# alperkartkaya2-afk/two-tower-augmented-with-adaptive-mimic-mechanism

Measured on AMD Instinct MI355X. Metric: training interactions/sec at 1/2/4/8 MI355X; Recall@20 parity vs CPU ref, higher is better.
Workload: dtype fp32

## Files before the change

two-tower-augmented-with-adaptive-mimic-mechanism_amd/csrc/gate.hip:

```cpp
#include <cstdlib>

#include "kernels.h"

namespace ttamm {

namespace {

typedef float f4v __attribute__((ext_vector_type(4)));
template <int D>
struct GateWaves {
    static constexpr int NW = D >= 128 ? 4 : 8;
    static constexpr int THREADS = 64 * NW;
};

__device__ __forceinline__ f4v ldg4(const float* p) { return *reinterpret_cast<const f4v*>(p); }
__device__ __forceinline__ f4v lds4(const float* p) { return *reinterpret_cast<const f4v*>(p); }
__device__ __forceinline__ void stg4(float* p, f4v v) { store_nt(p, make_float4(v[0], v[1], v[2], v[3])); }
__device__ __forceinline__ float sigmoid_(float x) { return 1.0f / (1.0f + __expf(-x)); }

template <int NO, int NK, int LD>
__device__ __forceinline__ void tile_gemm(const float* w_lds, int ob0, const f4v (&b)[NK], f4v (&acc)[NO], int li,
                                          int q) {
    f4v w[2][NO];
    const float* base = w_lds + (16 * ob0 + li) * LD + 4 * q;
// ... 37 lines not shown
                acc[ob] = __builtin_amdgcn_mfma_f32_16x16x4f32(w[cur][ob][r], b[t][r], acc[ob], 0, 0, 0);
        __builtin_amdgcn_sched_barrier(0);
    }
}

typedef __bf16 g_bf16x8 __attribute__((ext_vector_type(8)));
typedef __bf16 g_bf16x4 __attribute__((ext_vector_type(4)));
typedef float g_f32x8 __attribute__((ext_vector_type(8)));

__device__ __forceinline__ void split8(f4v a, f4v b, g_bf16x8& h, g_bf16x8& m, g_bf16x8& l) {
    const g_f32x8 x = {a[0], a[1], a[2], a[3], b[0], b[1], b[2], b[3]};
    h = __builtin_convertvector(x, g_bf16x8);
    const g_f32x8 r = x - __builtin_convertvector(h, g_f32x8);
    m = __builtin_convertvector(r, g_bf16x8);
    l = __builtin_convertvector(r - __builtin_convertvector(m, g_f32x8), g_bf16x8);
}

template <int NF>
__device__ __forceinline__ int xw_off(int t, int q, int f, int j) {
    return ((t * 4 + q) * NF + f) * 16 + j * 2;
}
__device__ __forceinline__ void xw_slot(int c, int& t, int& q, int& j) {
    t = c >> 5;
    const int r = c & 31;
    q = (r & 15) >> 2;
    j = ((r >> 4) << 2) | (r & 3);
}
template <int NF, int PLANE>
__device__ __forceinline__ void xw_store4(unsigned char* img, int t, int q, int f, int j0, f4v w) {
    const f4v hf = w;
    const g_bf16x4 h = __builtin_convertvector(hf, g_bf16x4);
    const f4v r = hf - __builtin_convertvector(h, f4v);
    const g_bf16x4 m = __builtin_convertvector(r, g_bf16x4);
    const g_bf16x4 l = __builtin_convertvector(r - __builtin_convertvector(m, f4v), g_bf16x4);
    const int off = xw_off<NF>(t, q, f, j0);
    *reinterpret_cast<g_bf16x4*>(img + off) = h;
    *reinterpret_cast<g_bf16x4*>(img + PLANE + off) = m;
    *reinterpret_cast<g_bf16x4*>(img + 2 * PLANE + off) = l;
}

template <int NO, int NT, int NF>
__device__ __forceinline__ void tile_gemm_x(const unsigned char* img, int ob0, const f4v* b, f4v (&acc)[NO], int li,
                                            int q) {
    constexpr int PLANE = NT * 4 * NF * 16;
#pragma unroll
    for (int t = 0; t < NT; ++t) {
        g_bf16x8 bh, bm, bl;
        split8(b[2 * t], b[2 * t + 1], bh, bm, bl);
        const unsigned char* base = img + xw_off<NF>(t, q, 16 * ob0 + li, 0);
#pragma unroll
        for (int ob = 0; ob < NO; ++ob) {
            const unsigned char* p = base + ob * 16 * 16;
            const g_bf16x8 ah = *reinterpret_cast<const g_bf16x8*>(p);
            const g_bf16x8 am = *reinterpret_cast<const g_bf16x8*>(p + PLANE);
            const g_bf16x8 al = *reinterpret_cast<const g_bf16x8*>(p + 2 * PLANE);
            acc[ob] = __builtin_amdgcn_mfma_f32_16x16x32_bf16(am, bm, acc[ob], 0, 0, 0);
            acc[ob] = __builtin_amdgcn_mfma_f32_16x16x32_bf16(al, bh, acc[ob], 0, 0, 0);
            acc[ob] = __builtin_amdgcn_mfma_f32_16x16x32_bf16(ah, bl, acc[ob], 0, 0, 0);
            acc[ob] = __builtin_amdgcn_mfma_f32_16x16x32_bf16(am, bh, acc[ob], 0, 0, 0);
            acc[ob] = __builtin_amdgcn_mfma_f32_16x16x32_bf16(ah, bm, acc[ob], 0, 0, 0);
            acc[ob] = __builtin_amdgcn_mfma_f32_16x16x32_bf16(ah, bh, acc[ob], 0, 0, 0);
        }
        __builtin_amdgcn_sched_barrier(0);
    }
}

template <int N>
__device__ __forceinline__ void zero(f4v (&a)[N]) {
#pragma unroll
    for (int i = 0; i < N; ++i) a[i] = f4v{0.f, 0.f, 0.f, 0.f};
}

template <int N>
__device__ __forceinline__ void load_row(f4v (&v)[N], const float* base, int64_t ld, int64_t row, int q) {
    const float* p = base + row * ld + 4 * q;
#pragma unroll
    for (int t = 0; t < N; ++t) v[t] = ldg4(p + 16 * t);
}

template <int D>
constexpr int slab_scratch() { return 8 * ((D < 96 ? 96 : D) + 4); }
template <int NO>
__device__ __forceinline__ void store_slab(float* scr, const f4v (&v)[NO], float* out, int64_t ld, int64_t row0,
                                           int64_t R, int lane) {
    constexpr int W = 16 * NO, LDW = W + 4, C4 = W / 4, PER = 8 * C4 / 64;
    static_assert((8 * C4) % 64 == 0, "slab scratch");
    const int li = lane & 15, q = lane >> 4;
#pragma unroll
    for (int half = 0; half < 2; ++half) {
        if ((li >> 3) == half) {
#pragma unroll
            for (int ob = 0; ob < NO; ++ob) *reinterpret_cast<f4v*>(scr + (li & 7) * LDW + 16 * ob + 4 * q) = v[ob];
        }
        __builtin_amdgcn_s_waitcnt(0xc07f);
        __builtin_amdgcn_wave_barrier();
#pragma unroll
        for (int k = 0; k < PER; ++k) {
            const int idx = lane + 64 * k, r = idx / C4, c = idx - r * C4;
            const f4v val = *reinterpret_cast<const f4v*>(scr + r * LDW + 4 * c);
            const int64_t grow = row0 + 8 * half + r;
            if (grow < R) stg4(out + grow * ld + 4 * c, val);
        }
        __builtin_amdgcn_s_waitcnt(0xc07f);
        __builtin_amdgcn_wave_barrier();
    }
}

template <int NO>
__device__ __forceinline__ void store_slab_xu(float* scr, const f4v (&v)[NO], float* out, int xu_li,
                                              bool pos_only, int64_t row0, int64_t R, int lane) {
    constexpr int W = 16 * NO, LDW = W + 4, C4 = W / 4, PER = 8 * C4 / 64;
    static_assert((8 * C4) % 64 == 0, "slab scratch");
    const int li = lane & 15, q = lane >> 4;
#pragma unroll
    for (int half = 0; half < 2; ++half) {
        if ((li >> 3) == half) {
#pragma unroll
            for (int ob = 0; ob < NO; ++ob) *reinterpret_cast<f4v*>(scr + (li & 7) * LDW + 16 * ob + 4 * q) = v[ob];
        }
        __builtin_amdgcn_s_waitcnt(0xc07f);
        __builtin_amdgcn_wave_barrier();
#pragma unroll
        for (int k = 0; k < PER; ++k) {
            const int idx = lane + 64 * k, r = idx / C4, c = idx - r * C4;
            const f4v val = *reinterpret_cast<const f4v*>(scr + r * LDW + 4 * c);
            const int64_t grow = row0 + 8 * half + r;
            const int u = __shfl(xu_li, 8 * half + r, 64);
            if (grow < R && (u >= 0 || !pos_only)) stg4(out + (int64_t)(u >= 0 ? u : ~u) * W + 4 * c, val);
        }
        __builtin_amdgcn_s_waitcnt(0xc07f);
        __builtin_amdgcn_wave_barrier();
    }
}

template <int N>
__device__ __forceinline__ void load_dt_row(f4v (&v)[N], const float* base, int64_t ld, const int64_t* xu, int D,
                                            int64_t row, int q) {
    if (xu) {
        const int64_t u = xu[row];
        load_row(v, base, D, u >= 0 ? u : ~u, q);
    } else {
        load_row(v, base, ld, row, q);
    }
}

template <int D, int HG, int NW_ = GateWaves<D>::NW>
struct GateCfg {
    static constexpr int TD = D / 16, TH = HG / 16, TE = 2 * D / 16;
    static constexpr int NW = NW_;
    static constexpr bool GG = D >= 128;
    static constexpr int SCR = slab_scratch<(D > HG ? D : HG)>();
    static constexpr int F_LD1 = 2 * D + 4, F_LD2 = HG + 4;
    static constexpr int F_LDS = HG * F_LD1 + (GG ? 0 : D * F_LD2) + HG + D;
    static constexpr int B_LD1 = D + 4, B_LD2 = HG + 4;
    static constexpr int B_G1T = GG ? 0 : HG * B_LD1;
    static constexpr int B_LDS = B_G1T + 2 * D * B_LD2;
    static_assert(D % 16 == 0 && HG % 16 == 0, "16-feature tiles");
    static_assert((F_LDS + NW * SCR) * 4 <= 163840 && (B_LDS + NW * SCR) * 4 <= 163840,
                  "the gate matrices must fit one CU's LDS");
    static constexpr int X1_BYTES = 3 * 2 * (2 * D) * HG;
    static constexpr int XF_BYTES = X1_BYTES + 4 * (D * F_LD2 + HG + D);
    static constexpr int XB_BYTES = X1_BYTES + 4 * (HG * B_LD1);
    static constexpr bool X_OK = !GG && (2 * D) % 32 == 0 && HG % 32 == 0 && XF_BYTES <= 163840 && XB_BYTES <= 163840;
};

__device__ __forceinline__ int gate_tower(const KArg(GateArgs) * ka, int& bidx) {
    bidx = blockIdx.x;
    if (ka->count > 1 && bidx >= ka->tw[0].blocks) {
        bidx -= ka->tw[0].blocks;
        return 1;
    }
    return 0;
}

template <int D, int HG, bool X, int NW>
__global__ __launch_bounds__(64 * NW) void gate_fwd_kernel(GateArgs) {
    using C = GateCfg<D, HG, NW>;
    constexpr int NT = 64 * NW;
    constexpr int NX = (2 * D) / 32;
    __shared__ __attribute__((aligned(16))) float lds[X ? C::XF_BYTES / 4 : C::F_LDS + NW * C::SCR];
    const KArg(GateArgs)* ka = (const KArg(GateArgs)*)(__builtin_amdgcn_kernarg_segment_ptr());
    int bidx;
    const KArg(GateTower)& T = ka->tw[gate_tower(ka, bidx)];
    float* g1s = lds;
// ... 19 lines not shown
#pragma unroll
    for (int e0 = 0; e0 < N1; e0 += NT) {
        const int e = e0 + (int)threadIdx.x;
        if (e < N1) {
            const int i = e / (2 * D / 4), c = 4 * (e % (2 * D / 4));
            const f4v w = ldg4(T.G1 + (int64_t)i * 2 * D + c);
            if constexpr (X) {
                int t, q4, j;
                xw_slot(c, t, q4, j);
                xw_store4<HG, C::X1_BYTES / 3>(img, t, q4, i, j, w);
            } else {
                *reinterpret_cast<f4v*>(g1s + i * C::F_LD1 + c) = w;
            }
        }
    }
    if constexpr (!C::GG) {
#pragma unroll
        for (int e0 = 0; e0 < N2; e0 += NT) {
            const int e = e0 + (int)threadIdx.x;
            if (e < N2) {
                const int i = e / (HG / 4), c = 4 * (e % (HG / 4));
                *reinterpret_cast<f4v*>(g2s + i * C::F_LD2 + c) = ldg4(T.G2 + (int64_t)i * HG + c);
            }
        }
    }
    for (int e = threadIdx.x; e < HG + D; e += NT) c1s[e] = e < HG ? T.c1[e] : T.c2[e - HG];
    __syncthreads();
    for (; s < nslab; s += stride) {
        const int64_t row = s * 16 + li;
        const bool ok = row < R;
        f4v a[C::TD];
        if (T.table) load_row(a, T.table, D, arow, q);
        const int xu_li = T.xu && ok ? (int)T.xu[row] : 0;
        f4v z[C::TH];
        zero(z);
        if constexpr (X) tile_gemm_x<C::TH, NX, HG>(img, 0, ef, z, li, q);
        else tile_gemm<C::TH, C::TE, C::F_LD1>(g1s, 0, ef, z, li, q);
        f4v nx[C::GG ? 1 : C::TE];
        int64_t arow_n = 0;
        const int64_t sn = s + stride;
        if (!C::GG && sn < nslab) {
            const int64_t rn = sn * 16 + li < R ? sn * 16 + li : R - 1;
            load_row(nx, T.ef, 2 * D, rn, q);
            if (T.table) arow_n = T.idx[rn];
        }
#pragma unroll
        for (int ob = 0; ob < C::TH; ++ob) {
            const f4v c1 = lds4(c1s + 16 * ob + 4 * q);
#pragma unroll
            for (int r = 0; r < 4; ++r) {
                const float v = z[ob][r] + c1[r];
                z[ob][r] = v > 0.f ? v : 0.f;
            }
            if ((X || (kDevKnobs && ka->direct)) && ok && !(kDevKnobs && ka->ablate)) stg4(T.z + row * HG + 16 * ob + 4 * q, z[ob]);
        }
        if (!(X || (kDevKnobs && ka->direct)) && !(kDevKnobs && ka->ablate)) store_slab<C::TH>(scr, z, T.z, HG, s * 16, R, lane);
        f4v x[C::TD];
        zero(x);
        if constexpr (C::GG) tile_gemm_g<C::TD, C::TH, HG>(T.G2, 0, z, x, li, q);
        else tile_gemm<C::TD, C::TH, C::F_LD2>(g2s, 0, z, x, li, q);
        if (!(X || (kDevKnobs && ka->direct)) && !(kDevKnobs && ka->ablate)) {
#pragma unroll
            for (int ob = 0; ob < C::TD; ++ob) {
                const f4v c2 = lds4(c2s + 16 * ob + 4 * q);
#pragma unroll
                for (int r = 0; r < 4; ++r) x[ob][r] = sigmoid_(x[ob][r] + c2[r]);
            }
            store_slab<C::TD>(scr, x, T.g, D, s * 16, R, lane);
#pragma unroll
            for (int ob = 0; ob < C::TD; ++ob) {
                const f4v e = ef[ob], f = ef[C::TD + ob];
#pragma unroll
                for (int r = 0; r < 4; ++r) x[ob][r] = x[ob][r] * e[r] + (1.0f - x[ob][r]) * f[r];
            }
            if (T.xu) {
                store_slab_xu<C::TD>(scr, a, T.a, xu_li, true, s * 16, R, lane);
                const bool neg = xu_li < 0;
#pragma unroll
                for (int ob = 0; ob < C::TD; ++ob)
#pragma unroll
                    for (int r = 0; r < 4; ++r) x[ob][r] = neg ? x[ob][r] + a[ob][r] : x[ob][r];
                store_slab_xu<C::TD>(scr, x, T.t, xu_li, false, s * 16, R, lane);
            } else {
                store_slab<C::TD>(scr, x, T.t, T.ld_t, s * 16, R, lane);
                if (T.table) {
                    store_slab<C::TD>(scr, a, T.a, T.ld_t, s * 16, R, lane);
#pragma unroll
                    for (int ob = 0; ob < C::TD; ++ob)
#pragma unroll
                        for (int r = 0; r < 4; ++r) x[ob][r] = x[ob][r] + a[ob][r];
                }
                if (T.aug) store_slab<C::TD>(scr, x, T.aug, D, s * 16, R, lane);
            }
        }
        if ((X || (kDevKnobs && ka->direct)) && ok && !(kDevKnobs && ka->ablate)) {
            const int64_t xu = xu_li;
            float* tdst = T.xu ? T.t + (xu >= 0 ? xu : ~xu) * D : T.t + row * T.ld_t;
            float* adst = T.xu ? (xu >= 0 ? T.a + xu * D : nullptr) : (T.table ? T.a + row * T.ld_t : nullptr);
#pragma unroll
            for (int ob = 0; ob < C::TD; ++ob) {
                const int col = 16 * ob + 4 * q;
                const f4v c2 = lds4(c2s + col);
                const f4v e = ef[ob], f = ef[C::TD + ob];
                f4v g, tt;
#pragma unroll
                for (int r = 0; r < 4; ++r) {
                    g[r] = sigmoid_(x[ob][r] + c2[r]);
                    tt[r] = g[r] * e[r] + (1.0f - g[r]) * f[r];
                }
                stg4(T.g + row * D + col, g);
                f4v aug = tt;
                if (T.table) {
#pragma unroll
                    for (int r = 0; r < 4; ++r) aug[r] = tt[r] + a[ob][r];
                }
                stg4(tdst + col, T.xu && xu < 0 ? aug : tt);
                if (adst) stg4(adst + col, a[ob]);
                if (T.aug) stg4(T.aug + row * D + col, aug);
            }
        }
        if constexpr (C::GG) {
            if (sn < nslab) {
                const int64_t rn = sn * 16 + li < R ? sn * 16 + li : R - 1;
                load_row(ef, T.ef, 2 * D, rn, q);
                if (T.table) arow = T.idx[rn];
            }
        } else if (sn < nslab) {
#pragma unroll
            for (int t = 0; t < C::TE; ++t) ef[t] = nx[t];
            arow = arow_n;
        }
    }
}

template <int D, int HG, bool X, int NW>
__global__ __launch_bounds__(64 * NW) void gate_bwd_kernel(GateArgs) {
    using C = GateCfg<D, HG, NW>;
    constexpr int NT = 64 * NW;
    constexpr int NX = HG / 32;
    __shared__ __attribute__((aligned(16))) float lds[X ? C::XB_BYTES / 4 : C::B_LDS + NW * C::SCR];
    const KArg(GateArgs)* ka = (const KArg(GateArgs)*)(__builtin_amdgcn_kernarg_segment_ptr());
    int bidx;
    const KArg(GateTower)& T = ka->tw[gate_tower(ka, bidx)];
    unsigned char* img = reinterpret_cast<unsigned char*>(lds);
    float* g2t = X ? reinterpret_cast<float*>(img + C::X1_BYTES) : lds;
    float* g1t = lds + C::B_G1T;
    float* scr = lds + C::B_LDS + (threadIdx.x >> 6) * C::SCR;
    const int lane = threadIdx.x & 63, wave = threadIdx.x >> 6;
    const int li = lane & 15, q = lane >> 4;
    const int64_t R = T.R;
    const int64_t nslab = (R + 15) / 16;
    const int64_t stride = (int64_t)T.blocks * NW;
    constexpr int N2 = D * (HG / 4), N1 = HG * (2 * D / 4);
    auto stage_g2t = [&]() {
#pragma unroll
        for (int e0 = 0; e0 < N2; e0 += NT) {
            const int e = e0 + (int)threadIdx.x;
            if (e < N2) {
                const int d = e / (HG / 4), j = 4 * (e % (HG / 4));
                const f4v v = ldg4(T.G2 + (int64_t)d * HG + j);
#pragma unroll
                for (int i = 0; i < 4; ++i) g2t[(j + i) * C::B_LD1 + d] = v[i];
            }
        }
    };
    if constexpr (C::GG) {
        for (int64_t s0 = (int64_t)bidx * NW; s0 < nslab; s0 += stride) {
            const int64_t s = s0 + wave;
            const bool has = s < nslab;
            const int64_t row = s * 16 + li;
            const bool ok = has && row < R;
            const int64_t rr = ok ? row : R - 1;
            f4v d[C::TD], g[C::TD], dz[C::TH];
            {
                f4v ef[C::TE];
                load_dt_row(d, T.dT, T.ld_dT, T.xu, D, rr, q);
                load_row(ef, T.ef, 2 * D, rr, q);
                load_row(g, T.g, D, rr, q);
                stage_g2t();
                __syncthreads();
                if (has) {
                    f4v dq[C::TD];
#pragma unroll
                    for (int t = 0; t < C::TD; ++t)
#pragma unroll
                        for (int r = 0; r < 4; ++r) {
                            const float dg = d[t][r] * ef[t][r] - d[t][r] * ef[C::TD + t][r];
                            dq[t][r] = dg * (1.0f - g[t][r]) * g[t][r];
                        }
                    if (!(kDevKnobs && ka->ablate)) store_slab<C::TD>(scr, dq, T.dq, D, s * 16, R, lane);
                    f4v zr[C::TH];
                    load_row(zr, T.z, HG, rr, q);
                    zero(dz);
                    tile_gemm<C::TH, C::TD, C::B_LD1>(g2t, 0, dq, dz, li, q);
#pragma unroll
                    for (int ob = 0; ob < C::TH; ++ob)
#pragma unroll
                        for (int r = 0; r < 4; ++r) dz[ob][r] = zr[ob][r] > 0.f ? dz[ob][r] : 0.f;
                    if (!(kDevKnobs && ka->ablate)) store_slab<C::TH>(scr, dz, T.dz, HG, s * 16, R, lane);
                }
            }
// ... 192 lines not shown
```

two-tower-augmented-with-adaptive-mimic-mechanism_amd/csrc/gemm.hip:

```cpp
#include <cstdlib>
#include <cstring>
#include <type_traits>

#include "kernels.h"

#ifndef TTAMM_GEMM_ABLATE
#define TTAMM_GEMM_ABLATE 0
#endif
#ifndef TTAMM_B16_ABLATE
#define TTAMM_B16_ABLATE 0
#endif

namespace ttamm {

typedef float f32x16 __attribute__((ext_vector_type(16)));
typedef float f32x8 __attribute__((ext_vector_type(8)));
typedef __bf16 bf16x8 __attribute__((ext_vector_type(8)));

namespace {


constexpr int BK = 16;
constexpr int SK = BK + 4;
constexpr int kThreads = 256;
constexpr int kWgradMaxRowsPerSplit = 1024;

__device__ __forceinline__ float sigmoidf_(float x) { return 1.0f / (1.0f + __expf(-x)); }
__device__ __forceinline__ bool aligned16(const void* p) { return (reinterpret_cast<uintptr_t>(p) & 15u) == 0; }
__device__ __forceinline__ bf16x8 pack_bf16(float4 a, float4 b) {
    const f32x8 v = {a.x, a.y, a.z, a.w, b.x, b.y, b.z, b.w};
    return __builtin_convertvector(v, bf16x8);
}
__device__ __forceinline__ float f4get(const float4& v, int q) {
    return q == 0 ? v.x : q == 1 ? v.y : q == 2 ? v.z : v.w;
}

__device__ __forceinline__ int clamp_col(int c, int ld) { return max(0, min(c, ld - 4)); }
__device__ __forceinline__ float4 raw4(const float* rp, int c, int ld) {
    return *reinterpret_cast<const float4*>(rp + clamp_col(c, ld));
}
__device__ __forceinline__ float4 mask4(float4 v, int c, int lim, int ld, int ones, bool ok) {
    const bool same = clamp_col(c, ld) == c;
    float t[4] = {v.x, v.y, v.z, v.w};
#pragma unroll
    for (int e = 0; e < 4; ++e) {
        const int ce = c + e;
        t[e] = (ok && same && ce < lim) ? t[e] : ((ok && ce == ones) ? 1.0f : 0.f);
    }
    return make_float4(t[0], t[1], t[2], t[3]);
}

template <int BM_, int BN_, int WAVES_M_, int WAVES_N_, bool A_KMAJ_, bool B_KMAJ_, int MF_ = 32>
struct Cfg {
    static constexpr int BM = BM_, BN = BN_, WAVES_M = WAVES_M_, WAVES_N = WAVES_N_, MF = MF_;
    static constexpr bool A_KMAJ = A_KMAJ_, B_KMAJ = B_KMAJ_;
    static constexpr int TM = BM / WAVES_M, TN = BN / WAVES_N;
    static constexpr int I = TM / MF, J = TN / MF;
    static constexpr int NR = MF == 32 ? 16 : 4;
    static constexpr int A_F4 = BM * BK / 4, B_F4 = BN * BK / 4;
    static constexpr int A_LOADS = (A_F4 + kThreads - 1) / kThreads;
    static constexpr int B_LOADS = (B_F4 + kThreads - 1) / kThreads;
    static constexpr int A_STAGE = A_KMAJ ? BK * BM : BM * SK;
    static constexpr int B_STAGE = B_KMAJ ? BK * BN : BN * SK;
    static constexpr int STAGE = 2 * (A_STAGE + B_STAGE);
    static constexpr int CLD = BN + 4;
    static constexpr int EPI_ROWS = WAVES_M >= 2 ? BM / 2 : (I > 1 ? (I + 1) / 2 * MF : BM);
    static constexpr int EPI_PHASES = (BM + EPI_ROWS - 1) / EPI_ROWS;
    static constexpr int EPI = EPI_ROWS * CLD;
    static constexpr int KIDX = A_KMAJ ? 2 * kWgradMaxRowsPerSplit : 0;
    static constexpr int LDS = (STAGE + KIDX) > EPI ? (STAGE + KIDX) : EPI;
    static_assert(WAVES_M * WAVES_N == 4, "4 waves per block");
    static_assert(MF == 32 || MF == 16, "MFMA block edge");
    static_assert(TM % MF == 0 && TN % MF == 0, "wave tile must be a multiple of the MFMA block");
    static_assert(WAVES_M == 1 || WAVES_M % EPI_PHASES == 0, "epilogue slices must hold whole wave rows");
};

__device__ __forceinline__ float4 ld4(const float* p) { return *reinterpret_cast<const float4*>(p); }
__device__ __forceinline__ void st4(float* p, float4 v) { store_nt(p, v); }

constexpr float kSeluAlpha = 1.6732632423543772848170429916717f;
constexpr float kSeluScale = 1.0507009873554804934193349852946f;
__device__ __forceinline__ float act_fwd(int act, float z) {
    switch (act) {
        case TTAMM_ACT_GELU: return z * 0.5f * (1.0f + erff(z * 0.70710678118654752440f));
        case TTAMM_ACT_TANH: return tanhf(z);
        case TTAMM_ACT_SELU: return z > 0.f ? z * kSeluScale : (expf(z) - 1.0f) * (kSeluAlpha * kSeluScale);
// ... 1142 lines not shown
        for (int i = 0; i < 4; ++i) {
            const int br = wm * 128 + i * 32;
            if (br < row_lo || br >= row_lo + kB16EpiRows) continue;
#pragma unroll
            for (int j = 0; j < 2; ++j)
#pragma unroll
                for (int r = 0; r < 16; ++r) {
                    const int rr = br - row_lo + (r & 3) + 8 * (r >> 2) + 4 * h;
                    Cs[rr * kB16Cld + wn * 64 + j * 32 + li] = acc[i][j][r];
                }
        }
        __syncthreads();
        if constexpr (E == EPI_HIDDEN) {
            constexpr int C4 = kB16N / 4;
            constexpr int RSTEP = kB16Threads / C4;
            static_assert(C4 % 2 == 0, "lane pairs hold 8-column groups");
            const int c4 = tid % C4, r0 = tid / C4;
            const int col = n0 + c4 * 4;
            if (r0 < RSTEP && col < ((N + 7) & ~7)) {
                const float4 bias4 = (P.bias && col < N) ? ld4(P.bias + col) : make_float4(0.f, 0.f, 0.f, 0.f);
                const float4 z4 = make_float4(0.f, 0.f, 0.f, 0.f);
#pragma unroll 2
                for (int rr = r0; rr < kB16EpiRows; rr += 2 * RSTEP) {
                    const int rb_ = rr + RSTEP;
                    const int ra = m0 + row_lo + rr, rb = m0 + row_lo + rb_;
                    const bool in_b = rb_ < kB16EpiRows;
                    epilogue_hidden_pair(P, ld4(Cs + rr * kB16Cld + c4 * 4), in_b ? ld4(Cs + rb_ * kB16Cld + c4 * 4) : z4, bias4,
                                         0, ra, rb, ra < M && col < N, in_b && rb < M && col < N, col);
                }
            }
        } else {
            constexpr int C4 = kB16N / 4;
            constexpr int RSTEP = kB16Threads / C4;
            const int c4 = tid % C4, r0 = tid / C4;
            const int col = n0 + c4 * 4;
            if (col < N) {
                const bool has_bias = (E == EPI_STORE || E == EPI_HIDDEN || E == EPI_GATE_HIDDEN || E == EPI_GATE_OUT) &&
                                      P.bias != nullptr;
                const float4 bias4 = has_bias ? ld4(P.bias + col) : make_float4(0.f, 0.f, 0.f, 0.f);
    #pragma unroll 2
                for (int rr = r0; rr < kB16EpiRows; rr += RSTEP) {
                    const int row = m0 + row_lo + rr;
    #if TTAMM_B16_ABLATE == 1
                    if (row < M) st4(P.C + (int64_t)row * P.ldc + col, ld4(Cs + rr * kB16Cld + c4 * 4));
    #else
                    if (row < M) epilogue4<E>(P, ld4(Cs + rr * kB16Cld + c4 * 4), bias4, 0, row, col);
    #endif
                }
            }
        }
        __syncthreads();
    }
}

__global__ void to_bf16_kernel(const float* __restrict__ src, int64_t rows, int cols, int64_t ld_src,
                               uint16_t* __restrict__ dst, int64_t ld_dst) {
    const int64_t total = rows * ld_dst;
    for (int64_t i = (int64_t)blockIdx.x * blockDim.x + threadIdx.x; i < total; i += (int64_t)gridDim.x * blockDim.x) {
        const int64_t r = i / ld_dst;
        const int c = (int)(i - r * ld_dst);
        const __bf16 v = (__bf16)(c < cols ? src[r * ld_src + c] : 0.f);
        dst[i] = __builtin_bit_cast(uint16_t, v);
    }
}

__global__ void to_planes_kernel(const float* __restrict__ src, int64_t rows, int cols, int64_t ld_src,
                                 uint16_t* __restrict__ dst, int64_t ld_dst, int kc) {
    const int64_t per_row = (int64_t)kc * 4;
    const int64_t total = rows * per_row;
    for (int64_t i = (int64_t)blockIdx.x * blockDim.x + threadIdx.x; i < total; i += (int64_t)gridDim.x * blockDim.x) {
        const int64_t r = i / per_row;
        const int g = (int)(i - r * per_row), c0 = 4 * g;
        float v[4];
#pragma unroll
        for (int e = 0; e < 4; ++e) v[e] = c0 + e < cols ? src[r * ld_src + c0 + e] : 0.f;
        uint2 w[3];
        split_bf16<3>(make_float4(v[0], v[1], v[2], v[3]), w);
        uint16_t* o = dst + r * ld_dst + (c0 >> 4) * 48 + (c0 & 15);
#pragma unroll
        for (int pl = 0; pl < 3; ++pl) *reinterpret_cast<uint2*>(o + 16 * pl) = w[pl];
    }
}

__global__ void wgrad_reduce_kernel(WgradBatch batch, int64_t total) {
    const KArg(WgradBatch)* kb = (const KArg(WgradBatch)*)(__builtin_amdgcn_kernarg_segment_ptr());
    const int64_t gid = (int64_t)blockIdx.x * blockDim.x + threadIdx.x;
    if (gid >= total) return;
    int64_t off = gid;
    int pi = 0;
    for (; pi < kb->count; ++pi) {
        const int64_t sz = (int64_t)kb->p[pi].M * (kb->p[pi].N + 1);
        if (off < sz) break;
        off -= sz;
    }
    const KArg(WgradProblem)& P = kb->p[pi];
    const int Mo = P.M;
    const int64_t plane = (int64_t)(P.N + 1) * Mo;
    const int n = (int)(off / Mo), m = (int)(off - (int64_t)n * Mo);
    float s = 0.f;
    const float* src = P.slab + off;
    int sp = 0;
    for (; sp + 8 <= P.splits; sp += 8) {
        float v[8];
#pragma unroll
        for (int i = 0; i < 8; ++i) v[i] = src[(int64_t)(sp + i) * plane];
#pragma unroll
        for (int i = 0; i < 8; ++i) s += v[i];
    }
    for (; sp < P.splits; ++sp) s += src[(int64_t)sp * plane];
    if (n < P.N) P.grad_w[(int64_t)m * P.N + n] = s;
    else if (P.grad_b) P.grad_b[m] = s;
}

template <class CF, int E, bool BF>
int launch_one(GemmBatch& b, hipStream_t s) {
    int tiles = 0;
    for (int i = 0; i < b.count; ++i) {
        GemmProblem& p = b.p[i];
        p.tiles_m = (int)ceil_div(p.M, CF::BM);
        p.tiles_n = (int)ceil_div(p.N, CF::BN);
        if (p.k_split <= 0) p.k_split = p.K;
        p.tile_begin = tiles;
        tiles += p.tiles_m * p.tiles_n * (int)ceil_div(p.K, p.k_split);
    }
    b.total_tiles = tiles;
    if (tiles == 0) return TTAMM_OK;
    hipLaunchKernelGGL((gemm_kernel<CF, E, BF>), dim3(tiles), dim3(kThreads), 0, s, b);
    TTAMM_LAUNCH_CHECK();
    return TTAMM_OK;
}

template <class CX, int E, int PL>
int launch_one_x(GemmBatch& b, hipStream_t s) {
    int tiles = 0;
    for (int i = 0; i < b.count; ++i) {
        GemmProblem& p = b.p[i];
        p.tiles_m = (int)ceil_div(p.M, CX::BM);
        p.tiles_n = (int)ceil_div(p.N, CX::BN);
        if (p.k_split <= 0) p.k_split = p.K;
        p.tile_begin = tiles;
        tiles += p.tiles_m * p.tiles_n * (int)ceil_div(p.K, p.k_split);
    }
    b.total_tiles = tiles;
    if (tiles == 0) return TTAMM_OK;
    hipLaunchKernelGGL((gemm_x_kernel<CX, E, PL>), dim3(tiles), dim3(kThreads), 0, s, b);
    TTAMM_LAUNCH_CHECK();
    return TTAMM_OK;
}
template <class CX, int PL>
int dispatch_epi_x(GemmBatch& b, hipStream_t s) {
    switch (b.p[0].epi) {
        case EPI_STORE: return launch_one_x<CX, EPI_STORE, PL>(b, s);
        case EPI_HIDDEN: return launch_one_x<CX, EPI_HIDDEN, PL>(b, s);
        case EPI_GATE_HIDDEN: return launch_one_x<CX, EPI_GATE_HIDDEN, PL>(b, s);
        case EPI_GATE_OUT: return launch_one_x<CX, EPI_GATE_OUT, PL>(b, s);
        case EPI_DGRAD_RELU: return launch_one_x<CX, EPI_DGRAD_RELU, PL>(b, s);
        case EPI_DGRAD_GATE_EF: return launch_one_x<CX, EPI_DGRAD_GATE_EF, PL>(b, s);
        case EPI_DGRAD_HIDDEN: return launch_one_x<CX, EPI_DGRAD_HIDDEN, PL>(b, s);
        default: return fail(TTAMM_E_INVALID, "gemm: unknown epilogue");
    }
}
template <int BM, int BN, int WM, int WN, bool AK, bool BK>
int dispatch_x(GemmBatch& b, hipStream_t s) {
    static const bool adeep2 = [] {
        const char* e = dev_env("TTAMM_GEMM_ADEEP");
        return e && e[0] == '2';
    }();
    if (b.p[0].bf16) return dispatch_epi_x<XCfg<BM, BN, WM, WN, AK, BK, 32>, 1>(b, s);
    if (adeep2 || AK || BK) return dispatch_epi_x<XCfg<BM, BN, WM, WN, AK, BK, 16>, 3>(b, s);
    return dispatch_epi_x<XCfg<BM, BN, WM, WN, AK, BK, 16, 3>, 3>(b, s);
}
int pick_tile_n(const GemmBatch& b, bool narrow, bool bf16) {
    static const bool legacy = [] {
        const char* e = dev_env("TTAMM_GEMM_TILES");
        return e && std::strcmp(e, "legacy") == 0;
    }();
    int maxN = 0;
    for (int i = 0; i < b.count; ++i) maxN = b.p[i].N > maxN ? b.p[i].N : maxN;
    if (maxN <= 96) return 96;
    if (legacy) return narrow ? 96 : 192;
    (void)bf16;
    static const int kNarrow[] = {96, 128};
    static const int kWide[] = {192, 128, 96};
    const int* c = narrow ? kNarrow : kWide;
    const int nc = narrow ? 2 : 3;
    int best = c[0];
    int64_t best_cols = -1;
    for (int j = 0; j < nc; ++j) {
        int64_t cols = 0;
        for (int i = 0; i < b.count; ++i) cols += ceil_div(b.p[i].M, 128) * ceil_div(b.p[i].N, c[j]) * c[j];
        if (best_cols < 0 || cols < best_cols) best_cols = cols, best = c[j];
    }
    return best;
}
// ... 164 lines not shown
                                 : (const void*)gemm_kernel<WgradNarrow, EPI_STORE, false>)
                          : cls == 0 ? (const void*)gemm_x_kernel<WgradNarrowX, EPI_STORE, 3>
                          : cls == 1 ? (const void*)gemm_x_kernel<WgradWideX, EPI_STORE, 3>
                                     : (const void*)gemm_x_kernel<Wgrad128X, EPI_STORE, 3>;
    if (hipOccupancyMaxActiveBlocksPerMultiprocessor(&per_cu, k, kThreads, 0) != hipSuccess || per_cu < 1) per_cu = 1;
    cached[exact][cls] = cus * per_cu;
    return cached[exact][cls];
}
constexpr int kWgradTileN[kWgradClasses] = {96, 192, 128, 128};
}

void wgrad_rows_per_split(const WgradShape* shapes, int n, int rps[kWgradClasses]) {
    if (const char* e = dev_env("TTAMM_WGRAD_ROWS_PER_SPLIT")) {
        const int v = std::atoi(e);
        if (v >= BK && v <= kWgradMaxRowsPerSplit && v % BK == 0) {
            for (int c = 0; c < kWgradClasses; ++c) rps[c] = v;
            return;
        }
    }
    const bool exact = exact_mfma();
    const double us_per_row[kWgradClasses] = {0.11, 0.14, 0.12, 0.12};
    const double hbm_us_per_byte = 1.0 / 5.0e6;
    for (int c = 0; c < kWgradClasses; ++c) {
        int best = 512;
        double best_cost = -1.0;
        for (int r = 128; r <= kWgradMaxRowsPerSplit; r += 32) {
            int64_t tiles = 0;
            double slab_bytes = 0.0;
            for (int i = 0; i < n; ++i) {
                if (shapes[i].R <= 0 || wgrad_class(shapes[i].M) != c) continue;
                const int64_t splits = ceil_div(shapes[i].R, r);
                tiles += ceil_div(shapes[i].N + 1, 128) * ceil_div(shapes[i].M, kWgradTileN[c]) * splits;
                slab_bytes += 2.0 * 4.0 * (double)splits * shapes[i].M * (shapes[i].N + 1);
            }
            if (tiles == 0) break;
            const double cost = (double)ceil_div(tiles, wgrad_slots(c, exact)) * r * us_per_row[c] +
                                slab_bytes * hbm_us_per_byte;
            if (best_cost < 0.0 || cost < best_cost) {
                best_cost = cost;
                best = r;
            }
        }
        rps[c] = best;
        if constexpr (kDevKnobs) {
            char name[] = "TTAMM_WGRAD_RPS0";
            name[sizeof(name) - 2] = (char)('0' + c);
            if (const char* e = dev_env(name)) {
                const int v = std::atoi(e);
                if (v >= BK && v <= kWgradMaxRowsPerSplit && v % BK == 0) rps[c] = v;
            }
        }
    }
}

size_t wgrad_slab_floats(int R, int M, int N, int rps) {
    const int splits = R > 0 ? (int)ceil_div(R, rps) : 1;
    return (size_t)splits * M * (N + 1);
}

int wgrad_class(int m_out) {
    static const bool all_narrow = dev_env("TTAMM_WGRAD_ALL_NARROW") != nullptr;
    static const bool legacy = [] {
        const char* e = dev_env("TTAMM_GEMM_TILES");
        return e && std::strcmp(e, "legacy") == 0;
    }();
    if (all_narrow || m_out <= 96) return 0;
    if (legacy) return 1;
    auto pad = [&](int bn) { return ceil_div(m_out, bn) * bn; };
    int best = 1;
    int64_t bp = pad(192);
    if (pad(256) < bp) best = 3, bp = pad(256);
    if (pad(128) < bp) best = 2, bp = pad(128);
    return best;
}

static bool wgrad_a3() {
    static const bool on = [] {
        const char* e = dev_env("TTAMM_WGRAD_ADEEP");
        return e && e[0] == '3';
    }();
    return on;
}

int launch_wgrad(WgradBatch& wb, hipStream_t s, void* const* ev) {
    GemmBatch g[kWgradClasses], gp[kWgradClasses];
    std::memset(g, 0, sizeof(g));
    std::memset(gp, 0, sizeof(gp));
    const bool bf = wb.count > 0 && wb.p[0].bf16;
    const bool exact = exact_mfma();
    const char* e256 = dev_env("TTAMM_BF16_WGRAD256");
    const bool w256 = e256 && e256[0] == '1';
    auto cfg_of = [&](int cls) {
        if (exact) return cls == 0 ? 0 : 1;
        if (bf && w256 && cls >= 2) return 3;
        return cls == 3 ? 2 : cls;
    };
    auto flush = [&](GemmBatch& b, int cfg, bool planes = false) -> int {
        if (b.count == 0) return TTAMM_OK;
        int rc;
        if (planes && bf) {
            rc = cfg == 1 ? launch_one_x<WgradWideX32A16, EPI_STORE, 1>(b, s)
                          : launch_one_x<Wgrad128X32A16, EPI_STORE, 1>(b, s);
        } else if (planes) {
            rc = cfg == 0   ? launch_one_x<WgradNarrowXP, EPI_STORE, 3>(b, s)
                 : cfg == 1 ? launch_one_x<WgradWideXP, EPI_STORE, 3>(b, s)
                            : launch_one_x<Wgrad128XP, EPI_STORE, 3>(b, s);
        } else if (exact) {
            rc = cfg ? (bf ? launch_one<WgradWide, EPI_STORE, true>(b, s) : launch_one<WgradWide, EPI_STORE, false>(b, s))
                     : (bf ? launch_one<WgradNarrow, EPI_STORE, true>(b, s) : launch_one<WgradNarrow, EPI_STORE, false>(b, s));
        } else if (bf) {
            rc = cfg == 0   ? launch_one_x<WgradNarrowX32, EPI_STORE, 1>(b, s)
                 : cfg == 1 ? launch_one_x<WgradWideX32, EPI_STORE, 1>(b, s)
                 : cfg == 3 ? launch_one_x<Wgrad256X32, EPI_STORE, 1>(b, s)
                            : launch_one_x<Wgrad128X32, EPI_STORE, 1>(b, s);
        } else {
            rc = cfg == 0   ? (wgrad_a3() ? launch_one_x<WgradNarrowXA3, EPI_STORE, 3>(b, s)
                                          : launch_one_x<WgradNarrowX, EPI_STORE, 3>(b, s))
                 : cfg == 1 ? launch_one_x<WgradWideX, EPI_STORE, 3>(b, s)
                            : launch_one_x<Wgrad128X, EPI_STORE, 3>(b, s);
        }
        std::memset(&b, 0, sizeof(b));
        return rc;
    };
    int64_t total = 0;
    for (int i = 0; i < wb.count; ++i) {
        WgradProblem& w = wb.p[i];
        TTAMM_REQUIRE(w.rows_per_split > 0 && w.rows_per_split % BK == 0 && w.rows_per_split <= kWgradMaxRowsPerSplit,
                      "wgrad: rows_per_split must be a multiple of 16 and at most 1024");
        TTAMM_REQUIRE(w.bf16 == wb.p[0].bf16, "wgrad: the batch must share one matmul precision");
        w.splits = w.R > 0 ? (int)ceil_div(w.R, w.rows_per_split) : 1;
        total += (int64_t)w.M * (w.N + 1);
        if (w.R <= 0) {
            TTAMM_HIP(hipMemsetAsync(w.slab, 0, sizeof(float) * w.M * (w.N + 1), s));
            continue;
        }
        TTAMM_REQUIRE(w.ld_x % 4 == 0 && w.ld_dy % 4 == 0 && ((uintptr_t)w.X | (uintptr_t)w.dY) % 16 == 0,
                      "wgrad: operands must be 16-byte aligned with leading dims % 4 == 0");
        GemmProblem p;
        std::memset(&p, 0, sizeof(p));
        p.A = w.X;
        p.a_idx = w.x_idx;
        p.lda = w.ld_x;
        p.a_kmaj = 1;
        p.a_cols = w.N;
        p.B = w.dY;
        p.ldb = w.ld_dy;
        p.b_kn = 1;
        p.b_colsum = 0;
        p.a_ones_col = w.N;
        p.M = w.N + 1;
        p.N = w.M;
        p.K = w.R;
        p.k_split = w.rows_per_split;
        p.epi = EPI_STORE;
        p.C = w.slab;
        p.ldc = w.M;
        p.slab_stride = (int64_t)(w.N + 1) * w.M;
        p.keep_prob = 1.f;
        p.inv_keep = 1.f;
        p.bf16 = w.bf16;
        const int cfg = cfg_of(wgrad_class(w.M));
        bool planes = w.X3p != nullptr && !exact && !bf && w.ld_x3 % 8 == 0 && (uintptr_t)w.X3p % 16 == 0 &&
                      w.ld_x3 >= 48 * ceil_div(w.N, 16);
        if (planes) {
            p.A3p = w.X3p;
            p.lda3 = w.ld_x3;
        }
        if (!exact && bf) {
            p.b_colsum = 1;
            p.a_ones_col = -1;
            p.M = w.N;
        }
        if (bf && w.X16 && (cfg == 1 || cfg == 2) && w.ld_x16 % 8 == 0 && w.ld_x16 >= 8 * ceil_div(w.N, 8) &&
            (uintptr_t)w.X16 % 16 == 0) {
            planes = true;
            p.A16 = w.X16;
            p.lda16 = w.ld_x16;
        }
        GemmBatch& gb = planes ? gp[cfg] : g[cfg];
        if (gb.count == kMaxGemmProblems) {
            const int rc = flush(gb, cfg, planes);
            if (rc) return rc;
        }
        gb.p[gb.count++] = p;
    }
    int rc;
    bool any_wide = false;
    for (int c = 1; c < kWgradClasses; ++c) any_wide = any_wide || g[c].count > 0 || gp[c].count > 0;
    const bool timed = ev && ev[0] && ev[1] && any_wide;
    static const bool narrow_first = dev_env("TTAMM_WGRAD_WIDE_FIRST") == nullptr;
    if (narrow_first && ((rc = flush(g[0], 0)) || (rc = flush(gp[0], 0, true)))) return rc;
    if (timed) TTAMM_HIP(hipEventRecord((hipEvent_t)ev[0], s));
    for (int c = 1; c < kWgradClasses; ++c)
        if ((rc = flush(gp[c], c, true)) || (rc = flush(g[c], c))) return rc;
    if (timed) TTAMM_HIP(hipEventRecord((hipEvent_t)ev[1], s));
    if (!narrow_first && ((rc = flush(g[0], 0)) || (rc = flush(gp[0], 0, true)))) return rc;
    if (total > 0) {
        hipLaunchKernelGGL(wgrad_reduce_kernel, dim3((unsigned)ceil_div(total, 256)), dim3(256), 0, s, wb, total);
        TTAMM_LAUNCH_CHECK();
    }
    return TTAMM_OK;
}

}
```

two-tower-augmented-with-adaptive-mimic-mechanism_amd/csrc/kernels.h:

```cpp
#pragma once

#include "common.h"

namespace ttamm {

enum Epilogue : int {
    EPI_STORE = 0,
    EPI_HIDDEN = 1,
    EPI_GATE_HIDDEN = 2,
    EPI_GATE_OUT = 3,
    EPI_DGRAD_RELU = 4,
    EPI_DGRAD_GATE_EF = 5,
    EPI_DGRAD_HIDDEN = 6,
};

struct GemmProblem {
    const float* A;
    const int64_t* a_idx;
    int64_t lda;
    const float* B;
    int64_t ldb;
    int b_kn;
    int M, N, K;
    int epi;
    float* C;
    int64_t ldc;
    const float* bias;
    const float* aux0;
    const float* aux1;
    const float* aux2;
    int64_t ld_aux0, ld_aux1, ld_aux2;
    float* out1;
    float* out2;
    float* out3;
    const float* table;
    const int64_t* idx;
    int64_t ld_out;
    int64_t ld_out2;
    float keep_prob;
    float inv_keep;
    const uint8_t* keep_mask;
    uint32_t rng_k0, rng_k1, rng_c2, rng_c3;
    const int64_t* row_key;
    int64_t key_base0, key_base1, key_split;
    int a_kmaj;
    int a_cols;
    int a_ones_col;
    int b_colsum;
    int k_split;
    int64_t slab_stride;
    int tile_begin;
    int tiles_m, tiles_n;
    int bf16;
    const uint16_t* A16;
    const uint16_t* B16;
    int64_t lda16;
    const uint16_t* A3p;
    int64_t lda3;
    int act;
    float* pre;
    uint8_t* mask_out;
};

constexpr int kMaxGemmProblems = 8;
struct GemmBatch {
    GemmProblem p[kMaxGemmProblems];
    int count;
    int total_tiles;
};

int launch_gemm(GemmBatch& batch, hipStream_t s);

int epoch_half_bits(int64_t n);
size_t route_scratch_bytes(int64_t n, int world);
int launch_route_rows(const int64_t* id0, int64_t n0, const int64_t* id1, int64_t n1, const int64_t* payload,
                      int64_t key0, int64_t key1, int world, int64_t* packed, int64_t* slot, int64_t* counts,
                      int64_t counts_ld, const uint32_t* status, void* scratch, size_t scratch_bytes, hipStream_t s);
void epoch_round_keys(uint64_t seed, int64_t epoch, uint32_t keys[4]);
int launch_epoch_batch(const int64_t* users, const int64_t* items, int64_t n, uint64_t seed, int64_t epoch,
                       int shuffle, int64_t start, int64_t count, int64_t* out_users, int64_t* out_items,
                       hipStream_t s);
int launch_to_bf16(const float* src, int64_t rows, int cols, int64_t ld_src, uint16_t* dst, int64_t ld_dst,
                   hipStream_t s);
int launch_to_planes(const float* src, int64_t rows, int cols, int64_t ld_src, uint16_t* dst, int64_t ld_dst,
                     hipStream_t s);

struct WgradProblem {
    const float* dY;
    int64_t ld_dy;
    const float* X;
    const int64_t* x_idx;
    int64_t ld_x;
    const uint16_t* X3p;
    int64_t ld_x3;
    const uint16_t* X16;
    int64_t ld_x16;
    int R, M, N;
    float* grad_w;
    float* grad_b;
    float* slab;
    int splits;
    int rows_per_split;
    int tile_begin;
    int tiles_m, tiles_n;
    int bf16;
};
constexpr int kMaxWgradProblems = 16;
static_assert(kMaxWgradProblems >= 2 * (TTAMM_MAX_LINEAR + 2), "both towers: every Linear + the gate's two");
struct WgradBatch {
    WgradProblem p[kMaxWgradProblems];
    int count;
    int total_blocks;
};
struct WgradShape {
    int64_t R;
    int M, N;
};
constexpr int kWgradClasses = 4;
int wgrad_class(int m_out);
void wgrad_rows_per_split(const WgradShape* shapes, int n, int rps[kWgradClasses]);
size_t wgrad_slab_floats(int R, int M, int N, int rows_per_split);
int launch_wgrad(WgradBatch& batch, hipStream_t s, void* const* ev = nullptr);

struct GateTower {
    int64_t R;
    const float* ef;
    const float* G1;
    const float* c1;
    const float* G2;
    const float* c2;
    float* z;
    float* g;
    float* t;
    float* a;
    int64_t ld_t;
    const float* table;
    const int64_t* idx;
    float* aug;
    const float* dT;
    int64_t ld_dT;
    const int64_t* xu;
    float* dq;
    float* dz;
    float* dEF;
    uint16_t* w16;
    int blocks;
};
struct GateArgs {
    GateTower tw[2];
    int count;
    int D, HG;
    int planes;
    int images_ready;
    int ablate;
    int direct;
};
bool gate_fused_supported(int D, int HG);
int launch_gate(GateArgs& a, bool backward, hipStream_t s);
bool gate16_supported(int D, int HG, int planes);
int64_t gate16_image_elems(int D, int HG, int planes);
int launch_gate16_prep(GateArgs& a, hipStream_t s);
int launch_gate16(GateArgs& a, bool backward, hipStream_t s);

int launch_renorm_rows(float* table, int64_t table_rows, int dim, const int64_t* idx, int64_t n, double max_norm,
                       int32_t* mark, int32_t tag, hipStream_t s, const int64_t* keys = nullptr,
                       int64_t key_split = 0, int key_phase = 0);
int launch_gather_rows(const float* table, int64_t table_rows, int dim, const int64_t* idx, int64_t n, float* out,
                       int64_t out_ld, hipStream_t s);

struct StageSeg {
    const int64_t* in;
    int64_t* out;
    int64_t n;
    int64_t rows;
    int64_t ld;
};
constexpr int kMaxStageSegs = 3;
struct StageArgs {
    StageSeg seg[kMaxStageSegs];
    int count;
    uint32_t* status;
    const int64_t* unit_counts;
    int64_t unit_ld;
    int unit_groups;
    int64_t unit_n;
    int64_t* unit_out;
};
int launch_stage_rows(const StageArgs& a, hipStream_t s);
int launch_add_rows(const float* x, int64_t ldx, const float* y, int64_t ldy, int64_t n, int dim, float* out,
                    int64_t ldo, hipStream_t s, const int64_t* xrow = nullptr);
int launch_scatter_add_rows(float* dst, int64_t dst_rows, int dim, const int64_t* idx, int64_t n, const float* x,
                            int64_t ldx, const float* y, int64_t ldy, const float* scale_dev, float scale,
                            int64_t skip_row, hipStream_t s);

constexpr uint32_t kStatusPoison =
    TTAMM_STATUS_SAMPLER_EXHAUSTED | TTAMM_STATUS_INDEX_OUT_OF_RANGE | TTAMM_STATUS_LOOKAHEAD_MISMATCH;
__device__ __forceinline__ bool step_poisoned(const uint32_t* status) {
    return status != nullptr && (*status & kStatusPoison) != 0u;
}
int launch_combine(const float* e, int64_t ld_e, const float* f, int64_t ld_f, const float* table,
                   int64_t table_rows, const int64_t* idx, int64_t n, int dim, float* t, float* a, int64_t ld_ta, float* aug,
                   hipStream_t s);
int launch_gate_mix(float* g, const float* ef, const float* table, const int64_t* idx, int64_t n, int dim, float* t,
                    float* a, int64_t ld_ta, float* aug, hipStream_t s);
int launch_pad_rows(const float* src, int64_t rows, int cols, int64_t ld_src, float* dst, int ld_dst,
                    hipStream_t s);
struct GatherSeg {
    const float* table;
    int64_t rows;
    int dim;
    const int64_t* idx;
    int64_t n;
    float* out;
    int64_t out_ld;
};
struct GatherSegs {
    GatherSeg seg[2];
    int count;
};
int launch_gather_rows_segs(const GatherSegs& g, hipStream_t s);
struct PadSeg {
    const float* src;
    int64_t rows;
    int cols;
    int64_t ld_src;
    float* dst;
    int ld_dst;
};
struct PadSegs {
    PadSeg seg[2];
    int count;
};
int launch_pad_rows_segs(const PadSegs& p, hipStream_t s);
int launch_mse(const float* x, const float* y, int64_t n, float* out, hipStream_t s);
int launch_gate_dq(const float* dT, int64_t ld_dT, const float* ef, const float* g, int64_t n, int dim,
                   float* dq, hipStream_t s);

struct ScoreArgs {
    int64_t B;
    int64_t Bg;
    int N;
    int D;
    const float* user_aug;
    const float* item_aug;
    const float* t_user;
    const float* t_item;
    const float* a_user;
    const float* a_item;
    int64_t ld_item;
    float lambda_u, lambda_i;
    int mimic;
    float* dT_user;
    float* dT_item;
    float* dA_user;
    float* dA_item;
    int dA_all;
    int neg_aug;
    int64_t ld_dti;
    const int64_t* item_slot;
    float* partials;
    int blocks;
    float inv_numel;
    const float* ib_du;
    const float* ib_dp;
    int64_t ib_ld;
};
int score_blocks(int64_t B, int D);
int launch_score_loss(const ScoreArgs& a, hipStream_t s);
struct EvalScoreArgs {
    int64_t B;
    int N;
    int D;
    const float* user_aug;
    const float* item_aug;
    int64_t ld_item;
    float* partials;
    int blocks;
    float* logits;
    int skip_pos;
};
int score_eval_check(int N, int D);
int launch_score_eval(const EvalScoreArgs& a, hipStream_t s);
int launch_eval_loss_finalize(const float* partials, int blocks, int64_t count, int64_t B, float* loss_out,
                              double* loss_accum, const uint32_t* status, hipStream_t s);
int launch_eval_loss_inbatch_finalize(const float* partials, int blocks, const float* ib_partials, int ib_blocks,
                                      int64_t count, int64_t B, float* loss_out, double* loss_accum,
                                      const uint32_t* status, hipStream_t s);
int launch_loss_finalize(const float* partials, int blocks, const float* ib_partials, int ib_blocks, int64_t bce_count,
                         int64_t B, int64_t Bg, int D, float lambda_u, float lambda_i, int mimic, const float* cal,
                         float lambda_cal, float* loss_out, double* loss_accum, const uint32_t* status, hipStream_t s);

struct InBatchArgs {
    const float* U;
    int64_t ldu, B;
    const float* P;
    int64_t ldp, Bc;
    int D;
    int64_t row_base;
    float inv_T;
    float* slab_u;
    float* slab_p;
    float* loss_part;
    float* dU;
    int64_t ld_du;
    float* dP;
    int64_t ld_dp;
    int rblk_u, rblk_p, splits_u, splits_p;
    int64_t cols_u, cols_p;
    const float* rmax;
    const float* rinv;
    float z_scale;
};
void inbatch_plan(int64_t B, int64_t Bc, InBatchArgs& a);
size_t inbatch_workspace_floats(int64_t B, int64_t Bc, int D, size_t* slab_u, size_t* slab_p, size_t* parts);
int launch_inbatch(InBatchArgs& a, hipStream_t s);
size_t inbatch_standalone_workspace_bytes(int64_t B, int64_t Bc, int D);
int inbatch_standalone(const float* U, int64_t B, int64_t ldu, const float* P, int64_t Bc, int64_t ldp, int D,
                       int64_t row_base, float inv_T, float* dU, int64_t ld_du, float* dP, int64_t ld_dp,
                       double* loss_sum, void* ws, size_t ws_bytes, hipStream_t s);
struct InBatchLossArgs {
    const float* U;
    int64_t ldu, B;
    const float* P;
    int64_t ldp, Bc;
    int D;
    int64_t row_base;
    float* loss_part;
// ... 73 lines not shown
    int32_t* lead_cnt;
    int32_t* seglong;
    int32_t* seg_start;
    int32_t* n_unique;
    int32_t* cnt;
    int32_t* first;
    int32_t* fill;
    int64_t key_range;
    int sorted;
};
constexpr int kCoalescePiece = 32;
size_t coalesce_scratch_ints(int64_t key_range);
void coalesce_bind_scratch(CoalesceWs& ws, int32_t* scratch, int64_t key_range);
int launch_coalesce_count(const int64_t* idx, int64_t n, int64_t table_rows, CoalesceWs& ws, hipStream_t s);
int launch_coalesce_group(const int64_t* idx, int64_t n, int64_t table_rows, CoalesceWs& ws, hipStream_t s);
int launch_coalesce(const int64_t* idx, int64_t n, int64_t table_rows, CoalesceWs& ws, hipStream_t s);

struct CalArgs {
    const float* x;
    int64_t ld_x;
    const float* xa;
    int64_t xa_rows;
    const int64_t* slot;
    const int64_t* idx;
    const int64_t* idx1;
    int64_t split;
    int64_t idx_rows;
    float* gstats;
    const int64_t* categories;
    int64_t num_categories;
    int64_t major;
    int64_t R;
    int D;
    float lambda;
    int64_t* catrow;
    CoalesceWs co;
    int nseg_max;
    int32_t* pcount;
    int32_t* pstart;
    float* psum;
    float* mean;
    float* pslab;
    float* cov;
    float* part;
    int32_t* flag;
    float* gmajor;
    float* out;
    float* dT;
    float* dA;
    int64_t ld_d;
    int64_t dA_rows;
};
int cal_max_pieces(int64_t R, int64_t nseg_max);
size_t cal_stats_floats(int64_t num_categories, int D);
size_t cal_scatter_floats(int64_t num_categories, int D);
int launch_cal_local(const CalArgs& a, hipStream_t s);
int launch_cal_scatter(const CalArgs& a, hipStream_t s);
int launch_cal_finish(const CalArgs& a, hipStream_t s);
int launch_block_exclusive_scan(const int32_t* in, int32_t* out, int64_t n, hipStream_t s);
int launch_category_alignment(const CalArgs& a, hipStream_t s);


struct AdamConsts {
    float decay;
    float w1;
    float b2;
    float w2;
    float eps;
    float neg_step;
    float bc2_sqrt;
    float inv_bc2_sqrt;
    float wd;
    float fast_ibc;
    float fast_eps;
    int decoupled;
    int fast_g0;
    int sgd;
    float sgd_neg_lr;
    float sgd_mom;
    float sgd_damp1;
    int sgd_first;
    int sgd_nesterov;
};
struct SparseConsts {
    float w1;
    float w2;
    float eps;
    float neg_step;
};

struct RowUpdateArgs {
    int64_t n;
    int dim;
    const int32_t* n_unique;
    const int32_t* seg_start;
    const int32_t* keys;
    const int32_t* rows;
    const int32_t* seglong;
    const float* dE;
    int64_t ld_dE;
    ttamm_table id;
    const float* dA_lo;
    const float* dA_hi;
    int64_t ld_dA;
    int64_t split_row;
    const int64_t* xu;
    ttamm_table mimic;
    float* piece_e;
    float* piece_a;
    float* side_id;
    float* side_mimic;
    SparseConsts sp;
    AdamConsts ad;
    int32_t dense_step;
    const uint32_t* status;
    const float* grad_scale;
    int lanes_per_row;
};
int launch_row_update(const RowUpdateArgs& a, hipStream_t s);
int rows_sumsq_blocks(int64_t n, int dim);
int launch_rows_sumsq(const RowUpdateArgs& a, float* partials, hipStream_t s);

constexpr int kMaxAdamHistory = 512;
int launch_step_begin(const uint32_t* status, int64_t* applied, AdamConsts* hist, int cap, int64_t step,
                      const AdamConsts& c, hipStream_t s);
struct ReplaySeg {
    float* p;
    float* m;
    float* v;
    int32_t* last;
    const uint8_t* touched;
    int dim;
    int64_t row_lo, row_hi;
    const int32_t* list_rows;
    const int32_t* list_lag;
    const int32_t* list_cnt;
};
constexpr int kMaxReplaySegs = 4;
struct ReplayArgs {
    ReplaySeg seg[kMaxReplaySegs];
    int count;
    const AdamConsts* hist;
    int cap;
    int32_t target;
    int stamp;
    int decoupled;
    int fast_g0;
    int sgd;
    const uint32_t* status;
};
int launch_replay(const ReplayArgs& a, hipStream_t s, void* const* ev = nullptr);

struct CatchupList {
    int32_t* cnt;
    int32_t* fill;
    int32_t* rows;
    int32_t* lag;
};
size_t catchup_list_ints(int64_t n, int cap);
void catchup_bind(CatchupList& cl, int32_t* ints, int64_t n, int cap);
int launch_catchup_list(const int64_t* idx, int64_t n, const int32_t* first, int32_t* const* last, int nlast,
                        int32_t target, int cap, const CatchupList& cl, const uint32_t* status, hipStream_t s);

struct PrepSeg {
    const int64_t* idx;
    int64_t n;
// ... 94 lines not shown
```

two-tower-augmented-with-adaptive-mimic-mechanism_amd/csrc/optim.hip:

```cpp
#include <algorithm>
#include <climits>
#include <cstdlib>
#include <cmath>
#include <cstring>

#include <type_traits>

#include "kernels.h"

#pragma clang fp contract(off)

namespace ttamm {

namespace {

template <bool DECOUPLED, bool G0 = false, bool FAST = false>
__device__ __forceinline__ void adam_elem_t(float& p, float& m, float& v, float g, const AdamConsts& c) {
    if (DECOUPLED) {
        p = p * c.decay;
    } else if (c.wd != 0.f) {
        g = g + p * c.wd;
    }
    if (G0 && DECOUPLED) {
        m = fmaf(c.w1, -m, m);
        v = v * c.b2;
    } else {
        m = fmaf(c.w1, g - m, m);
        v = v * c.b2;
        v = v + c.w2 * g * g;
    }
    if constexpr (FAST) {
        static_assert(G0, "fast arithmetic is for the g = 0 updates only");
        const float d = fmaf(__builtin_amdgcn_sqrtf(v), c.fast_ibc, c.fast_eps);
        p = fmaf(m, __builtin_amdgcn_rcpf(d), p);
    } else {
        const float denom = div_by_const(sqrtf(v), c.bc2_sqrt, c.inv_bc2_sqrt) + c.eps;
        p = p + c.neg_step * (m / denom);
    }
}

__device__ __forceinline__ void sgd_elem(float& p, float& m, float& v, float g, const AdamConsts& c) {
    if (c.wd != 0.f) g = fmaf(p, c.wd, g);
    if (c.sgd_mom != 0.f) {
        const float buf = c.sgd_first ? g : fmaf(g, c.sgd_damp1, m * c.sgd_mom);
        g = c.sgd_nesterov ? fmaf(buf, c.sgd_mom, g) : buf;
        p = fmaf(g, c.sgd_neg_lr, p);
        m = v = buf;
    } else {
        p = fmaf(g, c.sgd_neg_lr, p);
        m = v = p;
    }
}

__device__ __forceinline__ void adam_elem(float& p, float& m, float& v, float g, const AdamConsts& c) {
    if (c.sgd)
        sgd_elem(p, m, v, g, c);
    else if (c.decoupled)
        adam_elem_t<true>(p, m, v, g, c);
    else
        adam_elem_t<false>(p, m, v, g, c);
}
__device__ __forceinline__ void adam_elem_g0(float& p, float& m, float& v, const AdamConsts& c) {
    if (c.sgd) {
        sgd_elem(p, m, v, 0.f, c);
    } else if (c.fast_g0) {
        if (c.decoupled)
            adam_elem_t<true, true, true>(p, m, v, 0.f, c);
        else
            adam_elem_t<false, true, true>(p, m, v, 0.f, c);
    } else if (c.decoupled) {
        adam_elem_t<true, true>(p, m, v, 0.f, c);
    } else {
        adam_elem_t<false, true>(p, m, v, 0.f, c);
    }
}

__device__ __forceinline__ void sparse_adam_elem(float& p, float& m, float& v, float g, const SparseConsts& c) {
    const float om = m, ov = v;
    float um = (g - om) * c.w1;
    float uv = (g * g - ov) * c.w2;
    m = om + um;
    v = ov + uv;
    const float numer = um + om;
    const float denom = sqrtf(uv + ov) + c.eps;
    p = p + c.neg_step * (numer / denom);
}

__global__ void co_count_kernel(const int64_t* __restrict__ idx, int64_t n, int32_t* __restrict__ cnt,
                                int32_t* __restrict__ first) {
    const int64_t p = (int64_t)blockIdx.x * blockDim.x + threadIdx.x;
    if (p >= n) return;
    const int64_t key = idx[p];
    atomicAdd(&cnt[key], 1);
    atomicMax(&first[key], (int32_t)(INT_MAX - p));
}

__global__ void co_count_seg_kernel(PrepSegs) {
    const KArg(PrepSegs)* ka = (const KArg(PrepSegs)*)(__builtin_amdgcn_kernarg_segment_ptr());
    const KArg(PrepSeg)& S = ka->seg[blockIdx.y];
    if (blockIdx.x == 0 && S.list_cnt)
        for (int i = threadIdx.x; i < 2 * (ka->cap + 1); i += blockDim.x) S.list_cnt[i] = 0;
    const int64_t p = (int64_t)blockIdx.x * blockDim.x + threadIdx.x;
    if (p >= S.n) return;
    const int64_t key = S.idx[p];
    atomicAdd(&S.cnt[key], 1);
    atomicMax(&S.first[key], (int32_t)(INT_MAX - p));
}

__device__ __forceinline__ void co_entry(int by_key, int64_t i, const int64_t* __restrict__ idx,
                                         const int32_t* __restrict__ cnt, const int32_t* __restrict__ first,
                                         int32_t& f, int32_t& c) {
    if (by_key) {
        c = cnt[i];
        f = c > 0;
    } else {
        const int64_t key = idx[i];
        f = first[key] == (int32_t)(INT_MAX - i);
        c = f ? cnt[key] : 0;
    }
}

__device__ __forceinline__ void block_scan2(int32_t& f, int32_t& c, int32_t* sf, int32_t* sc) {
    const int t = threadIdx.x, lane = t & 63, w = t >> 6;
#pragma unroll
    for (int o = 1; o < 64; o <<= 1) {
        const int32_t a = __shfl_up(f, o, 64), b = __shfl_up(c, o, 64);
        if (lane >= o) {
            f += a;
            c += b;
        }
    }
    if (lane == 63) {
        sf[w] = f;
        sc[w] = c;
    }
    __syncthreads();
    int32_t pf = 0, pc = 0;
    for (int i = 0; i < w; ++i) {
        pf += sf[i];
        pc += sc[i];
    }
    f += pf;
    c += pc;
}

__global__ __launch_bounds__(256) void co_tile_sum_kernel(int64_t n, int by_key, const int64_t* __restrict__ idx,
                                                          const int32_t* __restrict__ cnt,
                                                          const int32_t* __restrict__ first,
                                                          int32_t* __restrict__ tile_f, int32_t* __restrict__ tile_c) {
    __shared__ int32_t sf[4], sc[4];
    const int64_t i = (int64_t)blockIdx.x * 256 + threadIdx.x;
    int32_t f = 0, c = 0;
    if (i < n) co_entry(by_key, i, idx, cnt, first, f, c);
    block_scan2(f, c, sf, sc);
    if (threadIdx.x == 255) {
        tile_f[blockIdx.x] = f;
        tile_c[blockIdx.x] = c;
    }
// ... 1390 lines not shown
```

two-tower-augmented-with-adaptive-mimic-mechanism_amd/csrc/rows.hip:

```cpp
#include "kernels.h"

namespace ttamm {

namespace {

__device__ __forceinline__ int64_t checked_row(int64_t r, int64_t rows) { return (r >= 0 && r < rows) ? r : -1; }

__global__ void gather_rows_vec4(const float* __restrict__ table, int64_t rows, int d4,
                                 const int64_t* __restrict__ idx, int64_t n, float* __restrict__ out, int64_t out_ld) {
    const int64_t total = n * d4;
    for (int64_t i = (int64_t)blockIdx.x * blockDim.x + threadIdx.x; i < total;
         i += (int64_t)gridDim.x * blockDim.x) {
        const int64_t r = i / d4;
        const int c = (int)(i - r * d4);
        const int64_t src = checked_row(idx[r], rows);
        float4 v = make_float4(0.f, 0.f, 0.f, 0.f);
        if (src >= 0) v = reinterpret_cast<const float4*>(table + src * (int64_t)d4 * 4)[c];
        reinterpret_cast<float4*>(out + r * out_ld)[c] = v;
    }
}

constexpr int cgcd(int a, int b) { return b == 0 ? a : cgcd(b, a % b); }
template <int D4>
struct WideGather {
// ... 114 lines not shown
    bool bad = false;
    for (int64_t i = (int64_t)blockIdx.x * blockDim.x + threadIdx.x; i < n; i += (int64_t)gridDim.x * blockDim.x) {
        const int64_t v = S.in[i * (S.ld ? S.ld : 1)];
        const bool ok = v >= 0 && v < rows;
        bad |= !ok;
        if (S.out) S.out[i] = ok ? v : 0;
    }
    if (ka->status && __ballot(bad) != 0ull && (threadIdx.x & 63) == 0)
        atomicOr(ka->status, TTAMM_STATUS_INDEX_OUT_OF_RANGE);
}

__global__ void combine_kernel(const float* __restrict__ e, int64_t ld_e, const float* __restrict__ f,
                               int64_t ld_f, const float* __restrict__ table, int64_t table_rows,
                               const int64_t* __restrict__ idx,
                               int64_t n, int dim, float* __restrict__ t, float* __restrict__ a, int64_t ld_ta,
                               float* __restrict__ aug) {
    const int64_t total = n * dim;
    for (int64_t i = (int64_t)blockIdx.x * blockDim.x + threadIdx.x; i < total;
         i += (int64_t)gridDim.x * blockDim.x) {
        const int64_t r = i / dim;
        const int c = (int)(i - r * dim);
        float tv = e[r * ld_e + c];
        if (f) tv = tv + f[r * ld_f + c];
        if (t) t[r * ld_ta + c] = tv;
        float av = tv;
        if (table) {
            const int64_t src = checked_row(idx[r], table_rows);
            const float am = src >= 0 ? table[src * (int64_t)dim + c] : 0.f;
            if (a) a[r * ld_ta + c] = am;
            av = tv + am;
        }
        if (aug) aug[i] = av;
    }
}

__global__ void pad_rows_kernel(const float* __restrict__ src, int64_t rows, int cols, int64_t ld_src,
                                float* __restrict__ dst, int ld_dst) {
    const int64_t total = rows * ld_dst;
    for (int64_t i = (int64_t)blockIdx.x * blockDim.x + threadIdx.x; i < total;
         i += (int64_t)gridDim.x * blockDim.x) {
        const int64_t r = i / ld_dst;
        const int c = (int)(i - r * ld_dst);
        dst[i] = c < cols ? src[r * ld_src + c] : 0.f;
    }
}

__global__ void pad_rows_seg_kernel(PadSegs) {
    const KArg(PadSegs)* ka = (const KArg(PadSegs)*)(__builtin_amdgcn_kernarg_segment_ptr());
    const KArg(PadSeg)& S = ka->seg[blockIdx.y];
    const int64_t total = S.rows * S.ld_dst;
    for (int64_t i = (int64_t)blockIdx.x * blockDim.x + threadIdx.x; i < total;
         i += (int64_t)gridDim.x * blockDim.x) {
        const int64_t r = i / S.ld_dst;
        const int c = (int)(i - r * S.ld_dst);
        S.dst[i] = c < S.cols ? S.src[r * S.ld_src + c] : 0.f;
    }
}

__global__ void gate_dq_kernel(const float* __restrict__ dT, int64_t ld_dT, const float* __restrict__ ef,
                               const float* __restrict__ g, int64_t n, int dim, float* __restrict__ dq) {
    const int64_t total = n * dim;
    for (int64_t i = (int64_t)blockIdx.x * blockDim.x + threadIdx.x; i < total;
         i += (int64_t)gridDim.x * blockDim.x) {
        const int64_t r = i / dim;
        const int c = (int)(i - r * dim);
        const float d = dT[r * ld_dT + c];
        const float ev = ef[r * 2 * dim + c], fv = ef[r * 2 * dim + dim + c];
        const float gv = g[i];
        const float dg = d * ev - d * fv;
        dq[i] = dg * (1.0f - gv) * gv;
    }
}

__device__ __forceinline__ float bce_logit(float x, float y) {
    const float m = fmaxf(-x, 0.f);
    return (1.0f - y) * x + m + logf(expf(-m) + expf(-x - m));
}

constexpr int kScoreWaves = 4;
constexpr int kMaxDChunks = 8;
constexpr int kMaxNeg = 64;

__device__ __forceinline__ float item_aug_at(const ScoreArgs& A, int64_t r, int d, bool neg = false) {
    if (A.item_aug) return A.item_aug[r * A.ld_item + d];
    const float t = A.t_item[r * A.ld_item + d];
    return A.a_item && !(neg && A.neg_aug) ? t + A.a_item[r * A.ld_item + d] : t;
}

constexpr int kScoreNG = 8;
template <int NCH>
__global__ __launch_bounds__(64 * kScoreWaves) void score_loss_kernel(ScoreArgs A) {
    __shared__ float red[kScoreWaves][3];
    const int lane = threadIdx.x & 63, w = threadIdx.x >> 6;
    const int64_t b = (int64_t)blockIdx.x * kScoreWaves + w;
    const int D = A.D, N = A.N;
    const int64_t B = A.B;
    const int64_t ldi = A.ld_dti;
    const float inv_numel = A.inv_numel;
    const bool ib = A.ib_du != nullptr;
    float bce = 0.f, mse_u = 0.f, mse_i = 0.f;
    if (b < B) {
        const int64_t pb = A.item_slot ? A.item_slot[b] : b;
        bool ok[NCH];
        float u[NCH], p[NCH], du[NCH], dpos[NCH];
        float au[NCH], tp[NCH], ap[NCH], tu[NCH], ibp[NCH], ibu[NCH];
#pragma unroll
        for (int c = 0; c < NCH; ++c) {
            const int d = c * 64 + lane;
            ok[c] = d < D;
            u[c] = p[c] = au[c] = tp[c] = ap[c] = tu[c] = ibp[c] = ibu[c] = 0.f;
            if (ok[c]) {
                u[c] = A.user_aug[b * D + d];
                p[c] = item_aug_at(A, pb, d);
                if (A.mimic) {
                    au[c] = A.a_user[b * D + d];
                    tp[c] = A.t_item[pb * A.ld_item + d];
                    ap[c] = A.a_item[pb * A.ld_item + d];
                    tu[c] = A.t_user[b * D + d];
                }
                if (ib) {
                    ibp[c] = A.ib_dp[b * A.ib_ld + d];
                    ibu[c] = A.ib_du[b * D + d];
                }
            }
        }
        float dot = 0.f;
#pragma unroll
        for (int c = 0; c < NCH; ++c)
            if (ok[c]) dot += u[c] * p[c];
        const float sp = wave_sum(dot);
        float dsp = 0.f;
        if (!ib) {
            dsp = (1.0f / (1.0f + expf(-sp)) - 1.0f) * inv_numel;
            bce += bce_logit(sp, 1.0f);
        }
#pragma unroll
        for (int c = 0; c < NCH; ++c) {
            const int d = c * 64 + lane;
            dpos[c] = 0.f;
            du[c] = 0.f;
            if (ok[c]) {
                dpos[c] = ib ? ibp[c] : dsp * u[c];
                A.dT_item[pb * ldi + d] = dpos[c];
                du[c] = ib ? ibu[c] : dsp * p[c];
            }
        }
        for (int j0 = 0; j0 < N; j0 += kScoreNG) {
            const int ng = N - j0 < kScoreNG ? N - j0 : kScoreNG;
            int64_t nr[kScoreNG];
            float nv[kScoreNG][NCH];
#pragma unroll
            for (int jj = 0; jj < kScoreNG; ++jj) {
                nr[jj] = 0;
                if (jj < ng) {
                    const int64_t q = B + b * N + j0 + jj;
                    nr[jj] = A.item_slot ? A.item_slot[q] : q;
                }
#pragma unroll
                for (int c = 0; c < NCH; ++c) nv[jj][c] = (jj < ng && ok[c]) ? item_aug_at(A, nr[jj], c * 64 + lane, true) : 0.f;
            }
            float sn[kScoreNG];
#pragma unroll
            for (int jj = 0; jj < kScoreNG; ++jj) {
                float dn = 0.f;
#pragma unroll
                for (int c = 0; c < NCH; ++c)
                    if (ok[c]) dn += u[c] * nv[jj][c];
                sn[jj] = jj < ng ? wave_sum(dn) : 0.f;
            }
#pragma unroll
            for (int jj = 0; jj < kScoreNG; ++jj) {
                if (jj >= ng) continue;
                const float dsn = (1.0f / (1.0f + expf(-sn[jj])) - 0.0f) * inv_numel;
                bce += bce_logit(sn[jj], 0.0f);
#pragma unroll
                for (int c = 0; c < NCH; ++c) {
                    const int d = c * 64 + lane;
                    if (ok[c]) {
                        const float g = dsn * u[c];
                        A.dT_item[nr[jj] * ldi + d] = g;
                        if (A.mimic && A.dA_all) A.dA_item[nr[jj] * ldi + d] = g;
                        du[c] += dsn * nv[jj][c];
                    }
                }
            }
        }
        const float norm = 2.0f / (float)(A.Bg * D);
#pragma unroll
        for (int c = 0; c < NCH; ++c) {
            const int d = c * 64 + lane;
            if (ok[c]) {
                A.dT_user[b * D + d] = du[c];
                if (A.mimic) {
                    const float xu = au[c] - tp[c], xi = ap[c] - tu[c];
                    mse_u += xu * xu;
                    mse_i += xi * xi;
                    A.dA_user[b * D + d] = du[c] + norm * xu * A.lambda_u;
                    A.dA_item[pb * ldi + d] = dpos[c] + norm * xi * A.lambda_i;
                }
            }
        }
        mse_u = wave_sum(mse_u);
        mse_i = wave_sum(mse_i);
    }
    if (lane == 0) {
        red[w][0] = bce;
        red[w][1] = mse_u;
        red[w][2] = mse_i;
    }
    __syncthreads();
    if (threadIdx.x < 3) {
        float s = 0.f;
        for (int i = 0; i < kScoreWaves; ++i) s += red[i][threadIdx.x];
        A.partials[blockIdx.x * 3 + threadIdx.x] = s;
    }
}

__device__ __forceinline__ float group_sum(float v, int G) {
    for (int o = G / 2; o > 0; o >>= 1) v += __shfl_xor(v, o, 64);
    return v;
}
__device__ __forceinline__ float dot4(float4 a, float4 b) { return a.x * b.x + a.y * b.y + a.z * b.z + a.w * b.w; }
__device__ __forceinline__ float4 scale4(float s, float4 a) { return make_float4(s * a.x, s * a.y, s * a.z, s * a.w); }
__device__ __forceinline__ float4 fma4(float s, float4 a, float4 c) {
    return make_float4(c.x + s * a.x, c.y + s * a.y, c.z + s * a.z, c.w + s * a.w);
}
__device__ __forceinline__ float4 ld4(const float* p) { return *reinterpret_cast<const float4*>(p); }
__device__ __forceinline__ void st4(float* p, float4 v) { *reinterpret_cast<float4*>(p) = v; }
__device__ __forceinline__ float4 addf4(float4 a, float4 b) { return make_float4(a.x + b.x, a.y + b.y, a.z + b.z, a.w + b.w); }

template <int G, int NV>
__global__ __launch_bounds__(64 * kScoreWaves) void score_loss_v_kernel(ScoreArgs A) {
    constexpr int NG = NV <= 3 ? 8 : 4;
    __shared__ float red[kScoreWaves][3];
    const int lane = threadIdx.x & 63, w = threadIdx.x >> 6, s = lane % G;
    const int64_t b = ((int64_t)blockIdx.x * kScoreWaves + w) * (64 / G) + lane / G;
    constexpr int D = 4 * G * NV;
    const int N = A.N;
    const int64_t B = A.B, ldi = A.ld_dti, ldt = A.ld_item;
    const float inv_numel = A.inv_numel;
    const bool ib = A.ib_du != nullptr;
    float bce = 0.f, mse_u = 0.f, mse_i = 0.f;
    if (b < B) {
        const int64_t pb = A.item_slot ? A.item_slot[b] : b;
        auto item_row = [&](int64_t r, int c, bool neg) {
            if (A.item_aug) return ld4(A.item_aug + r * ldt + c);
            const float4 t = ld4(A.t_item + r * ldt + c);
            return A.a_item && !(neg && A.neg_aug) ? addf4(t, ld4(A.a_item + r * ldt + c)) : t;
        };
        const float4 z4 = make_float4(0.f, 0.f, 0.f, 0.f);
        float4 u[NV], p[NV], au[NV], tp[NV], ap[NV], tu[NV], ibp[NV], ibu[NV];
#pragma unroll
        for (int i = 0; i < NV; ++i) {
            const int c = 4 * (s + G * i);
            u[i] = ld4(A.user_aug + b * D + c);
            p[i] = item_row(pb, c, false);
            au[i] = tp[i] = ap[i] = tu[i] = ibp[i] = ibu[i] = z4;
            if (A.mimic) {
                au[i] = ld4(A.a_user + b * D + c);
                tp[i] = ld4(A.t_item + pb * ldt + c);
                ap[i] = ld4(A.a_item + pb * ldt + c);
                tu[i] = ld4(A.t_user + b * D + c);
            }
            if (ib) {
                ibp[i] = ld4(A.ib_dp + b * A.ib_ld + c);
                ibu[i] = ld4(A.ib_du + b * D + c);
            }
        }
        float dot = 0.f;
#pragma unroll
        for (int i = 0; i < NV; ++i) dot += dot4(u[i], p[i]);
        const float sp = group_sum(dot, G);
        float dsp = 0.f;
        if (!ib) {
            dsp = (1.0f / (1.0f + expf(-sp)) - 1.0f) * inv_numel;
            bce += bce_logit(sp, 1.0f);
        }
        float4 du[NV], dpos[NV];
#pragma unroll
        for (int i = 0; i < NV; ++i) {
            dpos[i] = ib ? ibp[i] : scale4(dsp, u[i]);
            du[i] = ib ? ibu[i] : scale4(dsp, p[i]);
            st4(A.dT_item + pb * ldi + 4 * (s + G * i), dpos[i]);
        }
        for (int j0 = 0; j0 < N; j0 += NG) {
            const int ng = N - j0 < NG ? N - j0 : NG;
            int64_t nr[NG];
            float4 nv[NG][NV];
#pragma unroll
            for (int jj = 0; jj < NG; ++jj) {
                nr[jj] = 0;
                if (jj < ng) {
                    const int64_t q = B + b * N + j0 + jj;
                    nr[jj] = A.item_slot ? A.item_slot[q] : q;
                }
#pragma unroll
                for (int i = 0; i < NV; ++i) nv[jj][i] = jj < ng ? item_row(nr[jj], 4 * (s + G * i), true) : z4;
            }
            float sn[NG];
#pragma unroll
            for (int jj = 0; jj < NG; ++jj) {
                float dn = 0.f;
#pragma unroll
                for (int i = 0; i < NV; ++i) dn += dot4(u[i], nv[jj][i]);
                sn[jj] = group_sum(dn, G);
            }
#pragma unroll
            for (int jj = 0; jj < NG; ++jj) {
                if (jj >= ng) continue;
                const float dsn = (1.0f / (1.0f + expf(-sn[jj])) - 0.0f) * inv_numel;
                bce += bce_logit(sn[jj], 0.0f);
#pragma unroll
                for (int i = 0; i < NV; ++i) {
                    const int c = 4 * (s + G * i);
                    const float4 g = scale4(dsn, u[i]);
                    st4(A.dT_item + nr[jj] * ldi + c, g);
                    if (A.mimic && A.dA_all) st4(A.dA_item + nr[jj] * ldi + c, g);
                    du[i] = fma4(dsn, nv[jj][i], du[i]);
                }
            }
        }
        const float norm = 2.0f / (float)(A.Bg * D);
#pragma unroll
        for (int i = 0; i < NV; ++i) {
            const int c = 4 * (s + G * i);
            st4(A.dT_user + b * D + c, du[i]);
            if (A.mimic) {
                const float4 xu = make_float4(au[i].x - tp[i].x, au[i].y - tp[i].y, au[i].z - tp[i].z, au[i].w - tp[i].w);
                const float4 xi = make_float4(ap[i].x - tu[i].x, ap[i].y - tu[i].y, ap[i].z - tu[i].z, ap[i].w - tu[i].w);
                mse_u += dot4(xu, xu);
                mse_i += dot4(xi, xi);
                st4(A.dA_user + b * D + c, fma4(norm * A.lambda_u, xu, du[i]));
                st4(A.dA_item + pb * ldi + c, fma4(norm * A.lambda_i, xi, dpos[i]));
            }
        }
    }
    bce = wave_sum(s == 0 ? bce : 0.f);
    mse_u = wave_sum(mse_u);
// ... 643 lines not shown
```

two-tower-augmented-with-adaptive-mimic-mechanism_amd/csrc/step.hip:

```cpp
#include <algorithm>
#include <cstdint>
#include <cstdlib>
#include <cstring>
#include <vector>

#include "tower.h"

namespace ttamm {

namespace {

struct StepWs {
    TowerWs user, item;
    float* partials = nullptr;
    uint32_t* prologue_done = nullptr;
    int64_t* keys_own = nullptr;
    int64_t* own_units = nullptr;
    int score_blocks = 0;
    bool ib_on = false;
    InBatchArgs ib{};
    float* ib_du = nullptr;
    float* ib_dp = nullptr;
    int ib_parts = 0;
    bool ib_softmax = false;
// ... 467 lines not shown
    TowerWs* W[2] = {};
    AdamConsts ad{};
    SparseConsts sp{};
    Deferred df;
    explicit Step(const ttamm_step_args& a) : A(a) {}
};

int table_updates(const Step& c, const ttamm_tower* T[2], TowerWs* W[2], int n, const StreamPlan& pl, bool on_aux,
                  void* const events[2], const float* grad_scale = nullptr) {
    const int D = c.D;
    const bool mimic = c.mimic;
    const AdamConsts& ad = c.ad;
    const Deferred& df = c.df;
    const hipStream_t s = on_aux ? pl.aux : pl.s;
    int rc;
    if (!on_aux && (rc = join_grouping(pl))) return rc;
    for (int k = 0; k < n; ++k)
        if ((rc = tower_optimizer_rows(*T[k], *W[k], D, mimic, c.sp, ad, df, s, grad_scale))) return rc;
    if (df.on) {
        if (pl.slice) return TTAMM_OK;
        return replay_slice(T, n, mimic, df, df.step, 1, events, s);
    }
    SweepArgs sw;
    std::memset(&sw, 0, sizeof(sw));
    sw.ad = ad;
    sw.status = df.status;
    if (mimic)
        for (int k = 0; k < n; ++k) add_seg(sw, T[k]->mimic);
    for (int k = 0; k < n; ++k)
        if (T[k]->id.optimizer == TTAMM_OPT_DENSE) add_seg(sw, T[k]->id);
    const bool sweep = !(ad.sgd && ad.sgd_mom == 0.f && ad.wd == 0.f);
    if (events && events[0]) TTAMM_HIP(hipEventRecord((hipEvent_t)events[0], s));
    if (sweep && (rc = launch_dense_sweep(sw, s))) return rc;
    if (events && events[1]) TTAMM_HIP(hipEventRecord((hipEvent_t)events[1], s));
    for (int k = 0; k < n; ++k) {
        const ttamm_tower& t = *T[k];
        TowerWs& w = *W[k];
        if (mimic)
            if ((rc = launch_side_scatter(w.co.n_unique, w.co.keys_out, w.co.seg_start, w.side_mimic, w.R, D, t.mimic,
                                          df.status, s)))
                return rc;
        if (t.id.optimizer == TTAMM_OPT_DENSE)
            if ((rc = launch_side_scatter(w.co.n_unique, w.co.keys_out, w.co.seg_start, w.side_id, w.R, t.id.dim, t.id,
                                          df.status, s)))
                return rc;
    }
    return TTAMM_OK;
}

DenseAdamArgs dense_args(const ttamm_tower* T[2], TowerWs* W[2], const AdamConsts& ad, const uint32_t* status,
                         const float* grad_scale) {
    DenseAdamArgs da;
    std::memset(&da, 0, sizeof(da));
    da.ad = ad;
    da.status = status;
    da.grad_scale = grad_scale;
    auto add_dense = [&](float* p, float* m, float* v, const float* g, int64_t n) {
        da.t[da.count++] = DenseTensor{p, m, v, g, n};
    };
    for (int k = 0; k < 2; ++k) {
        const ttamm_tower& t = *T[k];
        TowerWs& w = *W[k];
        if (t.fusion == TTAMM_FUSION_IDENTITY) continue;
        for (int l = 0; l < t.n_linear; ++l) {
            const ttamm_linear& L = t.linear[l];
            add_dense(L.weight, L.weight_exp_avg, L.weight_exp_avg_sq, w.gw[l], (int64_t)L.out_features * L.in_features);
            add_dense(L.bias, L.bias_exp_avg, L.bias_exp_avg_sq, w.gb[l], L.out_features);
        }
        {
            for (int q = 0; q < fusion_linears(t); ++q) {
                const ttamm_linear& L = t.gate[q];
                add_dense(L.weight, L.weight_exp_avg, L.weight_exp_avg_sq, w.ggw[q],
                          (int64_t)L.out_features * L.in_features);
                add_dense(L.bias, L.bias_exp_avg, L.bias_exp_avg_sq, w.ggb[q], L.out_features);
            }
        }
    }
    return da;
}
int dense_update(const ttamm_tower* T[2], TowerWs* W[2], const AdamConsts& ad, const uint32_t* status, hipStream_t s,
                 const float* grad_scale = nullptr) {
    return launch_dense_adam(dense_args(T, W, ad, status, grad_scale), s);
}

int clip_table_partials(Step& c, const StreamPlan& pl, int* off_out) {
    StepWs& ws = c.ws;
    int rc;
    if ((rc = join_grouping(pl))) return rc;
    int off = 1;
    for (int k = 0; k < 2; ++k) {
        if (c.W[k]->R <= 0) continue;
        const RowUpdateArgs ru = row_update_args(*c.T[k], *c.W[k], c.D, c.mimic, c.sp, c.ad, c.df, nullptr);
        if ((rc = launch_rows_sumsq(ru, ws.clip_partials + off, pl.s))) return rc;
        off += rows_sumsq_blocks(c.W[k]->R, c.T[k]->id.dim);
    }
    TTAMM_REQUIRE(off <= ws.clip_parts, "clip: partials overflow");
    *off_out = off;
    return TTAMM_OK;
}

int clip_coefficient(Step& c, const StreamPlan& pl) {
    StepWs& ws = c.ws;
    int rc;
    int off;
    if ((rc = clip_table_partials(c, pl, &off))) return rc;
    if ((rc = launch_dense_sumsq(dense_args(c.T, c.W, c.ad, c.A.status, nullptr), ws.clip_partials + off, pl.s)))
        return rc;
    off += kDenseSumsqBlocks;
    TTAMM_REQUIRE(off <= ws.clip_parts, "clip: partials overflow");
    return launch_clip_coef(ws.clip_partials + 1, off - 1, (float)c.A.hp.grad_clip_norm, ws.clip_coef, pl.s);
}

int clip_table_share(Step& c, const StreamPlan& pl) {
    int rc;
    int off;
    if ((rc = clip_table_partials(c, pl, &off))) return rc;
    return launch_sum_partials(c.ws.clip_partials + 1, off - 1, c.A.table_sumsq, pl.s);
}

int clip_coefficient_sharded(Step& c, hipStream_t s) {
    StepWs& ws = c.ws;
    int rc;
    TTAMM_HIP(hipMemcpyAsync(ws.clip_partials, c.A.table_sumsq, sizeof(float), hipMemcpyDeviceToDevice, s));
    if ((rc = launch_dense_sumsq(dense_args(c.T, c.W, c.ad, c.A.status, nullptr), ws.clip_partials + 1, s))) return rc;
    return launch_clip_coef(ws.clip_partials, 1 + kDenseSumsqBlocks, (float)c.A.hp.grad_clip_norm, ws.clip_coef, s);
}

int deferred_of(const ttamm_step_args& A, Deferred& df) {
    const bool mimic = A.mimic_enabled != 0;
    int with = 0, total = 0;
    for (const ttamm_tower* t : {&A.user, &A.item}) {
        const ttamm_table* tabs[2];
        const int n = dense_tables(*t, mimic, tabs);
        for (int i = 0; i < n; ++i) {
            ++total;
            with += tabs[i]->last_step != nullptr ? 1 : 0;
        }
    }
    if (with == 0) return TTAMM_OK;
    TTAMM_REQUIRE(with == total, "deferred AdamW: every dense-group table needs last_step");
    TTAMM_REQUIRE(A.adam_history != nullptr && A.replay_slices >= 1 && A.history_capacity > A.replay_slices &&
                      A.history_capacity <= kMaxAdamHistory,
                  "deferred AdamW: needs adam_history and replay_slices < history_capacity <= 512");
    TTAMM_REQUIRE(A.hp.dense_step < (double)INT32_MAX, "deferred AdamW: step count out of range");
    df.on = true;
    df.hist = static_cast<AdamConsts*>(A.adam_history);
    df.cap = A.history_capacity;
    df.slices = A.replay_slices;
    df.step = (int32_t)A.hp.dense_step;
    df.decoupled = A.hp.decoupled_weight_decay ? 1 : 0;
    df.fast = A.table_g0_math == TTAMM_G0_FAST ? 1 : 0;
    df.sgd = A.hp.dense_optimizer == TTAMM_DENSE_SGD ? 1 : 0;
    return TTAMM_OK;
}

CalArgs& bind_cal(Step& st) {
    const ttamm_step_args& A = st.A;
    const TowerWs& I = st.ws.item;
    const int64_t B = st.B;
    const int D = st.D;
    const bool mimic = st.mimic;
    CalArgs& c = st.ws.cal;
    c.xa_rows = INT64_MAX;
    if (sharded(A)) {
        c.x = A.item_fwd_in;
        c.xa = mimic ? A.item_fwd_in + D : nullptr;
// ... 39 lines not shown
        c.dA = st.mimic ? st.ws.item.dA_own : nullptr;
        c.ld_d = D;
        c.dA_rows = st.B;
    }
    return c;
}

int64_t inbatch_cols(const Step& st) { return st.ws.ib_on ? (sharded(st.A) ? st.Bg : st.B) : 0; }
int64_t bce_count(const Step& st) {
    return st.ws.ib_softmax ? st.B : st.Bg * ((st.ws.ib_on ? inbatch_cols(st) : 1) + st.N);
}

InBatchArgs& bind_inbatch(Step& st) {
    const ttamm_step_args& A = st.A;
    const bool shard = sharded(A);
    const int D = st.D;
    InBatchArgs& a = st.ws.ib;
    a.U = st.ws.user.aug;
    a.ldu = D;
    a.B = st.B;
    a.P = shard ? A.inbatch_items : st.ws.item.aug;
    a.dP = shard ? A.inbatch_dp_all : st.ws.ib_dp;
    a.ldp = D;
    a.ld_dp = D;
    a.Bc = inbatch_cols(st);
    a.D = D;
    a.row_base = shard ? A.row_base : 0;
    a.inv_T = 1.0f / (float)bce_count(st);
    a.dU = st.ws.ib_du;
    a.ld_du = D;
    return a;
}
int run_inbatch(Step& st, hipStream_t s) {
    int rc;
    void* const* ev = st.A.timing_events + 4;
    if (ev[0] && ev[1]) TTAMM_HIP(hipEventRecord((hipEvent_t)ev[0], s));
    InBatchArgs& a = bind_inbatch(st);
    if (st.ws.ib_softmax) {
        InBatchLossArgs& l = st.ws.ib_lse;
        l.U = a.U, l.ldu = a.ldu, l.P = a.P, l.ldp = a.ldp, l.D = a.D, l.row_base = a.row_base;
        if ((rc = launch_inbatch_softmax(a, l, st.A.in_batch_inv_temperature, s))) return rc;
    } else if ((rc = launch_inbatch(a, s))) {
        return rc;
    }
    if (ev[0] && ev[1]) TTAMM_HIP(hipEventRecord((hipEvent_t)ev[1], s));
    return TTAMM_OK;
}

ScoreArgs bind_score(Step& st) {
    const ttamm_step_args& A = st.A;
    const TowerWs &U = st.ws.user, &I = st.ws.item;
    const int D = st.D;
    const bool mimic = st.mimic;
    ScoreArgs sa;
    std::memset(&sa, 0, sizeof(sa));
    sa.B = st.B;
    sa.Bg = st.Bg;
    sa.N = st.N;
    sa.D = D;
    sa.user_aug = U.aug;
    sa.t_user = U.t;
    sa.a_user = U.a;
    sa.lambda_u = (float)A.hp.lambda_mimic_user;
    sa.lambda_i = (float)A.hp.lambda_mimic_item;
    sa.mimic = mimic ? 1 : 0;
    sa.dT_user = U.dT_own;
    sa.dA_user = U.dA_own;
    if (sharded(A)) {
        sa.item_aug = nullptr;
        sa.t_item = A.item_fwd_in;
        sa.a_item = mimic ? A.item_fwd_in + D : nullptr;
        sa.ld_item = 2 * D;
        sa.dT_item = A.item_bwd_out;
        sa.dA_item = mimic ? A.item_bwd_out + D : nullptr;
        sa.dA_all = 1;
        sa.ld_dti = 2 * D;
        sa.item_slot = A.item_slot;
        if (compact_exchange(A)) {
            sa.ld_item = sa.ld_dti = D;
            sa.dA_all = 0;
            sa.neg_aug = 1;
        }
    } else {
        sa.item_aug = I.aug;
        sa.t_item = I.t;
        sa.a_item = I.a;
        sa.ld_item = D;
        sa.dT_item = I.dT_own;
        sa.dA_item = I.dA_own;
        sa.ld_dti = D;
    }
    sa.partials = st.ws.partials;
    sa.blocks = st.ws.score_blocks;
    sa.inv_numel = 1.0f / (float)bce_count(st);
    if (st.ws.ib_on) {
        sa.ib_du = st.ws.ib_du;
        sa.ib_dp = sharded(A) ? A.inbatch_dp : st.ws.ib_dp;
        sa.ib_ld = D;
    }
    return sa;
}

int loss_finalize(const Step& st, hipStream_t s) {
    const ttamm_step_args& A = st.A;
    const StepWs& ws = st.ws;
    if (!A.loss_out) return TTAMM_OK;
    const float* ib_part = ws.ib_softmax ? ws.ib_lse.loss_part : ws.ib_on ? ws.ib.loss_part : nullptr;
    const int ib_parts = ws.ib_softmax ? inbatch_lse_parts(st.B) : ws.ib_on ? ws.ib_parts : 0;
    return launch_loss_finalize(ws.partials, ws.score_blocks, ib_part, ib_parts, bce_count(st), st.B, st.Bg, st.D,
                                (float)A.hp.lambda_mimic_user, (float)A.hp.lambda_mimic_item, st.mimic ? 1 : 0,
                                ws.cal_on && A.row_base == 0 ? ws.cal.out : nullptr,
                                (float)A.hp.lambda_category_alignment, A.loss_out, A.loss_accum, A.status, s);
}

int validate_step(const ttamm_step_args& A) {
    const int D = out_dim(A.user);
    int rc;
    TTAMM_REQUIRE(A.table_g0_math == TTAMM_G0_EXACT || A.table_g0_math == TTAMM_G0_FAST,
                  "table_g0_math must be TTAMM_G0_EXACT or TTAMM_G0_FAST");
    if ((rc = validate_pair(A, true))) return rc;
    if (A.hp.grad_clip_norm > 0.0 && A.mimic_enabled)
        TTAMM_REQUIRE(A.user.id.dim == D && A.item.id.dim == D,
                      "gradient clipping with a concat output_dim other than the embedding dim is not supported");
    TTAMM_REQUIRE(A.b.batch > 0, "empty batch");
    if (cal_enabled(A)) {
        TTAMM_REQUIRE(!sharded(A) || (A.cal_stats && A.cal_scatter),
                      "the row-sharded category-alignment loss needs cal_stats and cal_scatter");
        TTAMM_REQUIRE(!sharded(A) || !(A.phase & (TTAMM_PHASE_CAL_STATS | TTAMM_PHASE_CAL_SCATTER |
                                                  TTAMM_PHASE_SCORE | TTAMM_PHASE_USER)) ||
                          (A.item_fwd_in && (A.b.num_neg == 0 || A.b.neg_items)),
                      "the row-sharded category-alignment loss needs item_fwd_in and b.neg_items");
        TTAMM_REQUIRE(A.num_categories > 0 && A.num_categories <= 65535,
                      "category alignment: num_categories must be in [1, 65535]");
        TTAMM_REQUIRE(A.major_category >= 0 && A.major_category < A.num_categories,
                      "category alignment: major_category out of range");
        TTAMM_REQUIRE(D <= 256, "category alignment: embedding dim must be <= 256");
    }
    TTAMM_REQUIRE(A.in_batch_loss == TTAMM_INBATCH_BCE || A.in_batch_loss == TTAMM_INBATCH_SOFTMAX,
                  "in_batch_loss must be 0 (the BCE mean) or 1 (the softmax cross-entropy)");
    if (A.in_batch_loss != TTAMM_INBATCH_BCE) {
        TTAMM_REQUIRE(!sharded(A),
                      "in_batch_loss: the softmax objective needs phase == 0, the whole step in one call (it is not "
                      "built for the row-sharded step)");
        TTAMM_REQUIRE(A.in_batch != 0, "in_batch_loss: the softmax objective needs in_batch");
        TTAMM_REQUIRE(A.b.num_neg == 0,
                      "in_batch_loss: the softmax objective needs b.num_neg == 0 (sampled negatives do not join the "
                      "denominator)");
        if ((rc = inbatch_softmax_check(A.in_batch_inv_temperature))) return rc;
    }
    if (A.in_batch) {
        TTAMM_REQUIRE(A.b.num_neg >= 0, "num_negatives must be >= 0 with in-batch negatives");
        TTAMM_REQUIRE(D % 4 == 0 && D <= 128, "in-batch negatives: embedding dim must be <= 128");
    } else {
        TTAMM_REQUIRE(A.b.num_neg > 0, "num_negatives must be greater than zero.");
    }
    const int64_t num_items = A.num_items_global > 0 ? A.num_items_global : A.item.id.rows;
    TTAMM_REQUIRE(num_items > 1, "num_items must be greater than one.");
    if ((rc = validate_mimic_pair(A))) return rc;
    TTAMM_REQUIRE(A.hp.dense_step >= 1 && A.hp.sparse_step >= 1, "optimizer step counts must be >= 1");
    TTAMM_REQUIRE(A.hp.dense_optimizer == TTAMM_DENSE_ADAM || A.hp.dense_optimizer == TTAMM_DENSE_SGD,
                  "hp.dense_optimizer must be TTAMM_DENSE_ADAM or TTAMM_DENSE_SGD");
    for (const ttamm_tower* t : {&A.user, &A.item})
        if (t->id.max_norm > 0.0) {
            TTAMM_REQUIRE(t->id.optimizer == TTAMM_OPT_DENSE, "max_norm is not supported when using sparse embeddings.");
        }
    if (A.hp.grad_clip_norm > 0.0) {
        TTAMM_REQUIRE(!sharded(A) || !(A.phase & (TTAMM_PHASE_USER | TTAMM_PHASE_ITEM_BWD)),
// ... 3 lines not shown
                      "gradient clipping needs dense ID tables (clip_grad_norm_ cannot take the sparse gradients "
                      "of sparse ID tables)");
    }
    TTAMM_REQUIRE(A.row_base >= 0 && (A.global_batch == 0 || A.global_batch >= A.row_base + A.b.batch),
                  "row_base / global_batch out of range");
    if (!sharded(A)) return TTAMM_OK;
    const int ph = A.phase;
    TTAMM_REQUIRE((ph & ~8191) == 0, "unknown phase bits");
    TTAMM_REQUIRE(!((ph & TTAMM_PHASE_USER) && (ph & (TTAMM_PHASE_SCORE | TTAMM_PHASE_TOWERS_BWD))),
                  "USER and SCORE / TOWERS_BWD are alternatives");
    TTAMM_REQUIRE(A.in_batch || (ph & (TTAMM_PHASE_INBATCH_SRC | TTAMM_PHASE_INBATCH)) == 0,
                  "INBATCH phases need in_batch");
    TTAMM_REQUIRE(A.item_rows_capacity >= 0 && A.n_item_rows >= 0 && A.n_item_rows <= A.item_rows_capacity,
                  "n_item_rows exceeds item_rows_capacity");
    if (ph & TTAMM_PHASE_SAMPLE)
        TTAMM_REQUIRE(!A.b.sample_negatives || A.b.neg_items, "sharded SAMPLE phase needs b.neg_items for the exchange");
    if (A.exchange_counts) {
        TTAMM_REQUIRE(A.mimic_enabled && A.item.fusion == TTAMM_FUSION_GATED,
                      "compact exchange rows (exchange_counts) need mimic on and a gated item tower");
        TTAMM_REQUIRE(A.exchange_world >= 1 && A.exchange_world <= 1024 && A.exchange_counts_ld >= 3,
                      "exchange_counts needs exchange_world in [1, 1024] and exchange_counts_ld >= 3");
        TTAMM_REQUIRE(A.item_slot, "compact exchange rows need item_slot (the requests' units)");
    }
    if ((ph & (TTAMM_PHASE_ITEM_FWD | TTAMM_PHASE_ITEM_BWD)) && A.n_item_rows > 0)
        TTAMM_REQUIRE(A.item_rows && A.item_row_keys, "item_rows / item_row_keys missing");
    if (ph & TTAMM_PHASE_ITEM_FWD) TTAMM_REQUIRE(A.item_fwd_out || A.n_item_rows == 0, "item_fwd_out missing");
    if (ph & (TTAMM_PHASE_USER | TTAMM_PHASE_SCORE))
        TTAMM_REQUIRE(A.item_fwd_in && A.item_bwd_out, "item_fwd_in / item_bwd_out missing");
    if (ph & (TTAMM_PHASE_ITEM_BWD | TTAMM_PHASE_TOWERS_BWD))
        TTAMM_REQUIRE(A.item_bwd_in || A.n_item_rows == 0, "item_bwd_in missing");
    if (ph & (TTAMM_PHASE_USER | TTAMM_PHASE_SCORE | TTAMM_PHASE_ITEM_BWD | TTAMM_PHASE_TOWERS_BWD |
              TTAMM_PHASE_DENSE))
        TTAMM_REQUIRE(A.dense_grads != nullptr, "dense_grads missing");
    return TTAMM_OK;
}

int bind_rows(Step& c) {
    const ttamm_step_args& A = c.A;
    int rc;
    if ((rc = validate_step(A))) return rc;
    const int D = c.D = out_dim(A.user);
    const bool mimic = c.mimic = A.mimic_enabled != 0;
    const bool shard = sharded(A);

    Arena ar{static_cast<char*>(A.workspace), A.workspace_bytes, 0, false};
    plan(ar, A, c.ws);
    TTAMM_REQUIRE(ar.ok(), "workspace too small for this step");

    const int64_t B = c.B = A.b.batch;
    const int N = c.N = A.b.num_neg;
    const int64_t Bg = c.Bg = global_batch(A);
    c.num_items = A.num_items_global > 0 ? A.num_items_global : A.item.id.rows;
    TowerWs& U = c.ws.user;
    TowerWs& I = c.ws.item;
    U.idx = U.fidx = U.idx_own;
    U.key_split = B;
    U.key_base0 = A.row_base;
    if (shard) {
        I.R = A.n_item_rows;
        I.idx = I.fidx = I.idx_own;
        I.row_key = c.ws.keys_own;
        I.t = A.item_fwd_out;
        I.a = mimic && A.item_fwd_out ? A.item_fwd_out + D : nullptr;
        I.t_ld = 2 * D;
        I.aug = nullptr;
        I.dT = A.item_bwd_in;
        I.dT_ld = 2 * D;
        I.dA = A.item_bwd_in ? A.item_bwd_in + D : nullptr;
        I.dA_ld = 2 * D;
        I.dA_split = I.R;
        if (compact_exchange(A)) {
            I.t_ld = I.dT_ld = I.dA_ld = D;
            I.xu = c.ws.own_units;
        }
        I.renorm_key_split = Bg;
        c.neg = A.b.neg_items;
    } else {
        I.idx = I.fidx = I.idx_own;
        I.key_split = B;
        I.key_base0 = A.row_base;
        I.key_base1 = Bg + A.row_base * N;
        c.neg = I.idx_own + B;
        I.renorm_split = B;
    }
    U.renorm_tag = I.renorm_tag = (int32_t)(2 * (A.hp.dense_step % (1 << 29)) + 1);
    c.T[0] = &A.user, c.T[1] = &A.item;
    c.W[0] = &U, c.W[1] = &I;
    const ttamm_hparams& hp = A.hp;
    c.ad = hp.dense_optimizer == TTAMM_DENSE_SGD
               ? make_sgd_consts(hp.lr, hp.weight_decay, hp.momentum, hp.dampening, hp.nesterov, hp.sgd_first_step)
               : make_adam_consts(hp.lr, hp.beta1, hp.beta2, hp.eps, hp.weight_decay, hp.decoupled_weight_decay,
                                  hp.dense_step);
    c.ad.fast_g0 = A.table_g0_math == TTAMM_G0_FAST ? 1 : 0;
    c.sp = make_sparse_consts(hp.sparse_lr, hp.sparse_beta1, hp.sparse_beta2, hp.sparse_eps, hp.sparse_step);
    if ((rc = deferred_of(A, c.df))) return rc;
    c.df.status = A.status;
    return TTAMM_OK;
}

int step_prologue(Step& c, bool begin_here, hipStream_t s) {
    const ttamm_step_args& A = c.A;
    const bool shard = sharded(A);
    const int64_t B = c.B;
    const int N = c.N;
    StageArgs st;
    std::memset(&st, 0, sizeof(st));
    st.status = A.status;
    st.seg[st.count++] = StageSeg{A.b.users, c.ws.user.idx_own, B, A.user.id.rows};
    if (!shard) {
        st.seg[st.count++] = StageSeg{A.b.pos_items, c.ws.item.idx_own, B, A.item.id.rows};
        if (!A.b.sample_negatives && N > 0) {
            TTAMM_REQUIRE(A.b.neg_items != nullptr, "negatives must be given when sample_negatives == 0");
            st.seg[st.count++] = StageSeg{A.b.neg_items, c.neg, B * N, A.item.id.rows};
        }
    } else {
        st.seg[st.count++] = StageSeg{A.b.pos_items, nullptr, B, c.num_items};
        if (!A.b.sample_negatives && A.b.neg_items && N > 0)
            st.seg[st.count++] = StageSeg{A.b.neg_items, nullptr, B * N, c.num_items};
    }
    TTAMM_REQUIRE(A.status != nullptr, "the training step needs a status word");
    TTAMM_REQUIRE(!(A.b.sample_negatives && N > 0) || c.num_items > 1, "num_items must be greater than one.");
    PrologueArgs pa;
    std::memset(&pa, 0, sizeof(pa));
    if (A.b.sample_negatives && N > 0) {
        pa.users = A.b.users;
        pa.user_rows = A.user.id.rows;
        pa.batch = B;
        pa.num_neg = N;
        pa.num_items = (uint64_t)c.num_items;
        pa.pos_offsets = A.b.pos_offsets;
        pa.pos_values = A.b.pos_values;
        pa.k0 = (uint32_t)A.b.seed;
        pa.k1 = (uint32_t)(A.b.seed >> 32);
        pa.counter = A.b.counter;
        pa.slot_base = A.row_base * N;
        pa.out = c.neg;
        pa.out2 = (!shard && A.b.neg_items != c.neg) ? A.b.neg_items : nullptr;
    }
    pa.cap = c.df.on ? c.df.cap : 2;
    pa.step = c.df.step;
    pa.c = c.ad;
    if (begin_here) {
        pa.done = c.ws.prologue_done;
        pa.applied = A.steps_applied;
        pa.hist = c.df.on ? c.df.hist : nullptr;
    }
    return launch_step_prologue(st, pa, s);
}

int rows_beside_mlp(Step& c, const StreamPlan& pl, bool single) {
    const ttamm_step_args& A = c.A;
    int rc;
    if ((rc = tower_backward(c.T, c.W, c.D, pl.s, 2, nullptr, BWD_GATE))) return rc;
    TTAMM_HIP(hipEventRecord(pl.ev[EV_TO_AUX], pl.s));
    TTAMM_HIP(hipStreamWaitEvent(pl.aux, pl.ev[EV_TO_AUX], 0));
    if (single && (rc = loss_finalize(c, pl.aux))) return rc;
    if ((rc = table_updates(c, c.T, c.W, 2, pl, true, A.timing_events))) return rc;
    TTAMM_HIP(hipEventRecord(pl.ev[EV_FROM_AUX], pl.aux));
    if ((rc = tower_backward(c.T, c.W, c.D, pl.s, 2, A.timing_events + 6, BWD_MLP))) return rc;
    if (single && (rc = dense_update(c.T, c.W, c.ad, A.status, pl.s))) return rc;
    TTAMM_HIP(hipStreamWaitEvent(pl.s, pl.ev[EV_FROM_AUX], 0));
    return TTAMM_OK;
}

int run_single(Step& c, const StreamPlan& pl) {
    const ttamm_step_args& A = c.A;
    const Deferred& df = c.df;
    StepWs& ws = c.ws;
    const hipStream_t s = pl.s;
    int rc;
    if ((rc = step_prologue(c, !pl.rows, s))) return rc;
    if ((rc = prepare_forward(c.T, c.W, 2, A.b, c.D, c.mimic, df, pl, A.timing_events + 2, A.timing_events,
                              A.timing_events + 8, A.timing_events + 12)))
        return rc;
    if (pl.rows && (rc = launch_step_begin(A.status, A.steps_applied, df.on ? df.hist : nullptr, df.on ? df.cap : 2,
                                           df.step, c.ad, pl.aux)))
        return rc;
    if (ws.ib_on && (rc = run_inbatch(c, s))) return rc;
    if ((rc = launch_score_loss(bind_score(c), s))) return rc;
    if (ws.cal_on && (rc = launch_category_alignment(bind_cal_grads(c), s))) return rc;
    if (pl.rows) return rows_beside_mlp(c, pl, true);
    if ((rc = loss_finalize(c, s))) return rc;
    if ((rc = tower_backward(c.T, c.W, c.D, s, 2, A.timing_events + 6))) return rc;
    if (ws.clip_on && (rc = clip_coefficient(c, pl))) return rc;
    if ((rc = table_updates(c, c.T, c.W, 2, pl, false, A.timing_events, ws.clip_coef))) return rc;
    return dense_update(c.T, c.W, c.ad, A.status, s, ws.clip_coef);
}

int phase_forward(Step& c, const StreamPlan& pl) {
    const ttamm_step_args& A = c.A;
    TowerWs& I = c.ws.item;
    const hipStream_t s = pl.s;
    const int ph = A.phase;
    int rc;
    if ((ph & TTAMM_PHASE_ITEM_FWD) && I.R > 0) {
        StageArgs st;
        std::memset(&st, 0, sizeof(st));
        st.status = A.status;
        st.seg[st.count++] = StageSeg{A.item_rows, I.idx_own, I.R, A.item.id.rows, A.item_rows_ld};
        st.seg[st.count++] = StageSeg{A.item_row_keys, c.ws.keys_own, I.R, INT64_MAX, A.item_rows_ld};
        if (compact_exchange(A)) {
            st.unit_counts = A.exchange_counts + (int64_t)A.exchange_world * A.exchange_counts_ld;
            st.unit_ld = A.exchange_counts_ld;
            st.unit_groups = A.exchange_world;
            st.unit_n = I.R;
            st.unit_out = c.ws.own_units;
        }
        if ((rc = launch_stage_rows(st, s))) return rc;
    }
    const ttamm_tower* Ti[2] = {&A.item, nullptr};
    TowerWs* Wi[2] = {&I, nullptr};
    const int both = TTAMM_PHASE_ITEM_FWD | TTAMM_PHASE_USER_FWD;
    if ((ph & both) == both && I.R > 0)
        return prepare_forward(c.T, c.W, 2, A.b, c.D, c.mimic, c.df, pl, A.timing_events + 2, nullptr,
                               A.timing_events + 8);
    if (ph & TTAMM_PHASE_ITEM_FWD) {
        if (I.R > 0) {
            if ((rc = prepare_forward(Ti, Wi, 1, A.b, c.D, c.mimic, c.df, pl, A.timing_events + 2, nullptr,
                                      A.timing_events + 8)))
                return rc;
        } else if ((rc = tower_prepare(A.item, I, c.mimic, c.df, s))) {
            return rc;
        }
    }
    if (ph & TTAMM_PHASE_USER_FWD)
        return prepare_forward(c.T, c.W, 1, A.b, c.D, c.mimic, c.df, pl, nullptr, nullptr, A.timing_events + 8);
    return TTAMM_OK;
}

int zero_item_grads(Step& c, hipStream_t s) {
    TowerWs& I = c.ws.item;
    const size_t n = tower_grad_floats(c.A.item);
    if (n) TTAMM_HIP(hipMemsetAsync(I.gw[0] ? I.gw[0] : I.ggw[0], 0, n * sizeof(float), s));
    return TTAMM_OK;
}

int run_phases(Step& c, const StreamPlan& pl) {
    const ttamm_step_args& A = c.A;
    StepWs& ws = c.ws;
    TowerWs& I = ws.item;
    const int D = c.D;
    const hipStream_t s = pl.s;
    const int ph = A.phase;
// ... 113 lines not shown
```

two-tower-augmented-with-adaptive-mimic-mechanism_amd/csrc/tower.h:

```cpp
#pragma once
#include <cstdint>

#include "kernels.h"

namespace ttamm {

enum Role { ROLE_USER = 0, ROLE_ITEM = 1 };

struct TowerWs {
    int role = ROLE_USER;
    int64_t R = 0;
    const int64_t* idx = nullptr;
    const int64_t* fidx = nullptr;
    int64_t* idx_own = nullptr;
    const int64_t* row_key = nullptr;
    int64_t key_base0 = 0, key_base1 = 0, key_split = 0;
    int32_t* renorm_mark = nullptr;
    int32_t renorm_tag = 0;
    int64_t renorm_split = 0;
    int64_t renorm_key_split = 0;
    float* hid[TTAMM_MAX_LINEAR] = {};
    float* dhid[TTAMM_MAX_LINEAR] = {};
    float* pre[TTAMM_MAX_LINEAR] = {};
    uint8_t* mask[TTAMM_MAX_LINEAR] = {};
    const uint8_t* keep[TTAMM_MAX_LINEAR] = {};
    float* ef = nullptr;
    float* e = nullptr;
    float* f = nullptr;
    float* z = nullptr;
    float* dz = nullptr;
    float* g = nullptr;
    float* t = nullptr;
    float* a = nullptr;
    int64_t t_ld = 0;
    float* aug = nullptr;
    const float* dT = nullptr;
    float* dT_own = nullptr;
    int64_t dT_ld = 0;
    const float* dA = nullptr;
    float* dA_own = nullptr;
    int64_t dA_ld = 0;
    int64_t dA_split = 0;
    const int64_t* xu = nullptr;
    float* dq = nullptr;
    float* dEF = nullptr;
    float* gw[TTAMM_MAX_LINEAR] = {};
    float* gb[TTAMM_MAX_LINEAR] = {};
    float* ggw[2] = {};
    float* ggb[2] = {};
    float* slab[TTAMM_MAX_LINEAR + 2] = {};
    CoalesceWs co{};
    CatchupList cl{};
    float* side_id = nullptr;
    float* side_mimic = nullptr;
    float* piece_e = nullptr;
    float* piece_a = nullptr;
    float* wpad = nullptr;
    uint16_t* w16 = nullptr;
    uint16_t* gw16 = nullptr;
    bool gw16_ready = false;
    int wgrad_rps[kWgradClasses] = {512, 512, 512, 512};
};

inline int round4(int x) { return (x + 3) / 4 * 4; }
inline int round8(int x) { return (x + 7) / 8 * 8; }
inline bool uses_w16(const ttamm_tower& T) {
    return T.matmul_bf16 && T.features_bf16 != nullptr && T.fusion != TTAMM_FUSION_IDENTITY && T.n_linear > 0;
}
inline bool uses_ef(const ttamm_tower& T) { return T.fusion == TTAMM_FUSION_GATED || T.fusion == TTAMM_FUSION_CONCAT; }
inline int fusion_linears(const ttamm_tower& T) {
    return T.fusion == TTAMM_FUSION_GATED ? 2 : T.fusion == TTAMM_FUSION_CONCAT ? 1 : 0;
}
inline int fo_dim(const ttamm_tower& T) { return T.n_linear ? T.linear[T.n_linear - 1].out_features : T.feat_dim; }
inline int efw(const ttamm_tower& T) { return T.id.dim + fo_dim(T); }
inline int out_dim(const ttamm_tower& T) { return T.fusion == TTAMM_FUSION_CONCAT ? T.gate[0].out_features : T.id.dim; }
inline bool needs_wpad(const ttamm_tower& T) {
    return T.fusion != TTAMM_FUSION_IDENTITY && T.n_linear > 0 && T.linear[0].in_features % 4 != 0;
}

int validate_tower(const ttamm_tower& T, const char* name, int D, bool training);
int validate_pair(const ttamm_step_args& A, bool training);
int validate_mimic_pair(const ttamm_step_args& A);

enum { IO_T = 1, IO_AUG = 2, IO_DT = 4, IO_ALL = 7 };
struct TowerPlan {
    bool backward = false;
    int io = 0;
    bool mimic = false;
    int64_t dA_rows = 0;
    bool w16 = false;
    bool gw16 = false;
    bool claim_marks = false;
    bool f_any = false;
};
void plan_tower(Arena& ar, const ttamm_tower& T, int64_t R, const TowerPlan& o, TowerWs& w);

size_t tower_grad_floats(const ttamm_tower& T);
void carve_grads(const ttamm_tower& T, TowerWs& w, float*& cur);
int wgrad_shapes(const ttamm_tower& T, int64_t R, WgradShape* out);

bool gate_choice(const ttamm_tower* const* T, const bool* has16, int ntowers, int D, int& hg, int& planes);

enum { FWD_GATHER = 1, FWD_FUSION = 2, FWD_FEAT = 4, FWD_MLP = FWD_GATHER | FWD_FEAT, FWD_ALL = 7 };
int tower_forward(const ttamm_tower* T[2], TowerWs* W[2], const ttamm_batch& bt, int D, bool mimic, hipStream_t s,
                  int ntowers, void* const* l0_events = nullptr, int part = FWD_ALL, hipEvent_t after_l0 = nullptr);
enum { BWD_GATE = 1, BWD_MLP = 2, BWD_ALL = 3 };
int tower_backward(const ttamm_tower* T[2], TowerWs* W[2], int D, hipStream_t s, int ntowers,
                   void* const* wg_events = nullptr, int part = BWD_ALL);

int stage_ids(const StageSeg* segs, int nsegs, uint32_t* status, const ttamm_tower* const* T, TowerWs* const* W,
              int ntowers, hipStream_t s);
int tower_forward_eval_mode(const ttamm_tower* const* T, TowerWs* const* W, int ntowers, int D, bool mimic,
                            hipStream_t s);

}
```

two-tower-augmented-with-adaptive-mimic-mechanism_amd/csrc/tower.hip:

```cpp
#include <cstdint>
#include <cstring>
#include <string>

#include "tower.h"

namespace ttamm {

namespace {
int tower_in_dim(const ttamm_tower& T, int l) { return l == 0 ? T.feat_dim : T.linear[l - 1].out_features; }
}

int validate_tower(const ttamm_tower& T, const char* name, int D, bool training) {
    std::string n(name);
    TTAMM_REQUIRE(T.id.weight, n + ": embedding table missing");
    if (training) TTAMM_REQUIRE(T.id.exp_avg && T.id.exp_avg_sq, n + ": embedding optimizer state missing");
    TTAMM_REQUIRE(T.fusion == TTAMM_FUSION_CONCAT || T.id.dim == D, n + ": embedding dim mismatch");
    TTAMM_REQUIRE(D % 4 == 0 && T.id.dim % 4 == 0, n + ": ttamm requires embedding_dim % 4 == 0");
    TTAMM_REQUIRE(T.id.rows > 0, n + ": empty embedding table");
    TTAMM_REQUIRE(T.id.rows < (int64_t(1) << 31), n + ": tables of 2^31 rows or more are not supported (int32 row keys)");
    TTAMM_REQUIRE(T.n_linear >= 0 && T.n_linear <= TTAMM_MAX_LINEAR, n + ": too many feature-encoder layers");
    TTAMM_REQUIRE(T.activation >= TTAMM_ACT_RELU && T.activation <= TTAMM_ACT_SELU, n + ": unsupported activation");
    TTAMM_REQUIRE(T.fusion >= TTAMM_FUSION_IDENTITY && T.fusion <= TTAMM_FUSION_CONCAT, n + ": unsupported fusion");
    if (T.fusion != TTAMM_FUSION_IDENTITY) {
        TTAMM_REQUIRE(T.features != nullptr && T.feat_dim > 0, n + ": fusion needs feature rows");
        TTAMM_REQUIRE(T.feat_ld >= T.feat_dim, n + ": feature row stride too small");
        TTAMM_REQUIRE(T.id.rows < (int64_t(1) << 31), n + ": feature rows of 2^31 rows or more are not supported "
                                                          "(the weight gradient gathers them by int32 row ids)");
        TTAMM_REQUIRE(T.feat_ld % 4 == 0 && (uintptr_t)T.features % 16 == 0,
                      n + ": feature rows must be 16-byte aligned (row stride % 4 == 0)");
        if (T.features_bf16)
            TTAMM_REQUIRE(T.matmul_bf16 && T.feat_bf16_ld % 8 == 0 && T.feat_bf16_ld >= round8(T.feat_dim) &&
                              (uintptr_t)T.features_bf16 % 16 == 0,
                          n + ": bf16 feature rows need matmul_bf16, 16-byte aligned rows of >= round8(F) elements");
        if (T.features_planes)
            TTAMM_REQUIRE(!T.matmul_bf16 && T.feat_planes_ld % 8 == 0 &&
                              T.feat_planes_ld >= 48 * ceil_div(T.feat_dim, 16) && (uintptr_t)T.features_planes % 16 == 0,
                          n + ": feature planes need fp32 GEMMs and 16-byte aligned rows of >= 48 ceil(F / 16) "
                              "elements (a multiple of 8)");
        for (int l = 0; l < T.n_linear; ++l) {
            const ttamm_linear& L = T.linear[l];
            TTAMM_REQUIRE(L.weight && L.bias, n + ": linear parameters missing");
            if (training)
                TTAMM_REQUIRE(L.weight_exp_avg && L.weight_exp_avg_sq && L.bias_exp_avg && L.bias_exp_avg_sq,
                              n + ": linear optimizer state missing");
            TTAMM_REQUIRE(L.in_features == tower_in_dim(T, l), n + ": feature-encoder layer shapes do not chain");
            TTAMM_REQUIRE(L.out_features % 4 == 0, n + ": ttamm requires feature-encoder widths % 4 == 0");
        }
        const int fo = fo_dim(T);
        if (T.fusion == TTAMM_FUSION_CONCAT)
            TTAMM_REQUIRE(fo % 4 == 0, n + ": ttamm requires the feature encoder's output width % 4 == 0");
        else
            TTAMM_REQUIRE(fo == D, n + ": Feature encoder output dimension must match id embedding dimension for "
                                       "'sum' or 'gated' fusion.");
        TTAMM_REQUIRE(T.dropout >= 0.f && T.dropout < 1.f, n + ": dropout must be in [0, 1)");
    }
    if (T.fusion == TTAMM_FUSION_GATED) {
        const ttamm_linear &G1 = T.gate[0], &G2 = T.gate[1];
        TTAMM_REQUIRE(G1.weight && G1.bias && G2.weight && G2.bias, n + ": gate parameters missing");
        if (training)
            TTAMM_REQUIRE(G1.weight_exp_avg && G1.weight_exp_avg_sq && G1.bias_exp_avg && G1.bias_exp_avg_sq &&
                              G2.weight_exp_avg && G2.weight_exp_avg_sq && G2.bias_exp_avg && G2.bias_exp_avg_sq,
                          n + ": gate optimizer state missing");
        TTAMM_REQUIRE(G1.in_features == 2 * D && G2.out_features == D && G2.in_features == G1.out_features,
                      n + ": gate shapes do not match the embedding dimension");
        TTAMM_REQUIRE(G1.out_features % 4 == 0, n + ": ttamm requires the gate hidden width % 4 == 0");
    }
    if (T.fusion == TTAMM_FUSION_CONCAT) {
        const ttamm_linear& P = T.gate[0];
        TTAMM_REQUIRE(P.weight && P.bias, n + ": concat projection parameters missing");
        if (training)
            TTAMM_REQUIRE(P.weight_exp_avg && P.weight_exp_avg_sq && P.bias_exp_avg && P.bias_exp_avg_sq,
                          n + ": concat projection optimizer state missing");
        TTAMM_REQUIRE(P.in_features == efw(T) && P.out_features == D,
                      n + ": concat projection must map [e | f] (embedding dim + feature output) to the output dim");
    }
    return TTAMM_OK;
}

int validate_pair(const ttamm_step_args& A, bool training) {
    const int D = out_dim(A.user);
    int rc;
    if ((rc = validate_tower(A.user, "user_encoder", D, training))) return rc;
// ... 134 lines not shown
};

void set_dropout(GemmProblem& p, const ttamm_tower& T, const ttamm_batch& bt, int tower_id, int layer,
                 const uint8_t* mask) {
    const float pdrop = T.dropout;
    p.keep_prob = 1.0f - pdrop;
    p.inv_keep = pdrop > 0.f ? 1.0f / (1.0f - pdrop) : 1.0f;
    p.keep_mask = mask;
    p.rng_k0 = (uint32_t)bt.seed;
    p.rng_k1 = (uint32_t)(bt.seed >> 32);
    p.rng_c2 = (uint32_t)bt.counter;
    p.rng_c3 = RNG_DROPOUT | ((uint32_t)tower_id << 24) | ((uint32_t)layer << 20) |
               ((uint32_t)(bt.counter >> 32) & 0xFFFFFu);
}

void set_keys(GemmProblem& p, const TowerWs& w) {
    p.row_key = w.row_key;
    p.key_base0 = w.key_base0;
    p.key_base1 = w.key_base1;
    p.key_split = w.key_split;
}

bool generic_gate_forced() {
    const char* v = product_env("TTAMM_GENERIC_GATE");
    return v && v[0] == '1';
}
}

bool gate_choice(const ttamm_tower* const* T, const bool* has16, int ntowers, int D, int& hg, int& planes) {
    hg = planes = -1;
    if (generic_gate_forced()) return false;
    const char* e16 = dev_env("TTAMM_GATE16_SPLIT");
    const bool split16 = e16 && e16[0] == '1';
    for (int k = 0; k < ntowers; ++k) {
        const ttamm_tower& t = *T[k];
        if (t.fusion != TTAMM_FUSION_GATED) continue;
        const int h = t.gate[0].out_features;
        int np;
        if (t.matmul_bf16) {
            if (!(gate16_supported(D, h, 1) && has16[k])) return false;
            np = 1;
        } else if (split16 && gate16_supported(D, h, 3) && has16[k]) {
            np = 3;
        } else if (gate_fused_supported(D, h)) {
            np = 0;
        } else {
            return false;
        }
        if ((hg >= 0 && h != hg) || (planes >= 0 && np != planes)) return false;
        hg = h;
        planes = np;
    }
    return hg >= 0;
}

namespace {
bool gate_group(const ttamm_tower* const* T, TowerWs* const* W, int ntowers, int D, bool mimic, GateArgs& ga) {
    std::memset(&ga, 0, sizeof(ga));
    bool has16[2] = {};
    for (int k = 0; k < ntowers; ++k) has16[k] = W[k]->gw16 != nullptr;
    int hg, planes;
    if (!gate_choice(T, has16, ntowers, D, hg, planes)) return false;
    ga.planes = planes;
    ga.images_ready = 1;
    for (int k = 0; k < ntowers; ++k) {
        const ttamm_tower& t = *T[k];
        const TowerWs& w = *W[k];
        if (t.fusion != TTAMM_FUSION_GATED || w.R <= 0) continue;
        GateTower& g = ga.tw[ga.count++];
        g.R = w.R;
        g.ef = w.ef;
        g.G1 = t.gate[0].weight;
        g.c1 = t.gate[0].bias;
        g.G2 = t.gate[1].weight;
        g.c2 = t.gate[1].bias;
        g.z = w.z;
        g.g = w.g;
        g.t = w.t;
        g.a = w.a;
        g.ld_t = w.t_ld;
        g.table = mimic ? t.mimic.weight : nullptr;
        g.idx = w.idx;
        g.aug = w.aug;
        g.dT = w.dT;
        g.ld_dT = w.dT_ld;
        g.dq = w.dq;
        g.dz = w.dz;
        g.dEF = w.dEF;
        g.xu = w.xu;
        g.w16 = w.gw16;
        if (!w.gw16_ready) ga.images_ready = 0;
    }
    ga.D = D;
    ga.HG = hg;
    return true;
}

int require_fused_for_units(const ttamm_tower* const* T, TowerWs* const* W, int ntowers, bool fused_gate) {
    for (int k = 0; k < ntowers; ++k)
        TTAMM_REQUIRE(!W[k]->xu || (T[k]->fusion == TTAMM_FUSION_GATED && fused_gate),
                      "compact exchange rows (exchange_counts) need the item tower on the fused gate kernels "
                      "(ttamm_exchange_compact_supported)");
    return TTAMM_OK;
}

bool gate_out_epilogue() {
    static const bool on = dev_env("TTAMM_GATE_OUT_EPILOGUE") != nullptr;
    return on;
}
int forward_fusion(const ttamm_tower* T[2], TowerWs* W[2], int D, bool mimic, hipStream_t s, int ntowers);
}

int tower_forward(const ttamm_tower* T[2], TowerWs* W[2], const ttamm_batch& bt, int D, bool mimic, hipStream_t s,
                  int ntowers, void* const* l0_events, int part, hipEvent_t after_l0) {
    int rc;
    if (part & FWD_GATHER) {
        GatherSegs gs;
        gs.count = 0;
        for (int k = 0; k < ntowers; ++k) {
            const ttamm_tower& t = *T[k];
            TowerWs& w = *W[k];
            if (t.id.max_norm > 0.0 && w.R > 0 && w.row_key && w.renorm_key_split > 0) {
                for (int ph = 0; ph < 2; ++ph)
                    if ((rc = launch_renorm_rows(t.id.weight, t.id.rows, t.id.dim, w.idx, w.R, t.id.max_norm, w.renorm_mark,
                                                 w.renorm_tag + ph, s, w.row_key, w.renorm_key_split, ph)))
                        return rc;
            } else if (t.id.max_norm > 0.0 && w.R > 0) {
                const int64_t split = w.renorm_split > 0 && w.renorm_split < w.R ? w.renorm_split : w.R;
                if ((rc = launch_renorm_rows(t.id.weight, t.id.rows, t.id.dim, w.idx, split, t.id.max_norm, w.renorm_mark,
                                             w.renorm_tag, s)))
                    return rc;
                if (split < w.R &&
                    (rc = launch_renorm_rows(t.id.weight, t.id.rows, t.id.dim, w.idx + split, w.R - split, t.id.max_norm,
                                             w.renorm_mark, w.renorm_tag + 1, s)))
                    return rc;
            }
            float* dst = uses_ef(t) ? w.ef : w.e;
            const int64_t ld = uses_ef(t) ? efw(t) : t.id.dim;
            gs.seg[gs.count++] = GatherSeg{t.id.weight, t.id.rows, t.id.dim, w.idx, w.R, dst, ld};
        }
        if ((rc = launch_gather_rows_segs(gs, s))) return rc;
    }
    if (part & FWD_FEAT) {
        for (int k = 0; k < ntowers; ++k) {
            const ttamm_tower& t = *T[k];
            TowerWs& w = *W[k];
            if (t.fusion != TTAMM_FUSION_IDENTITY && t.n_linear == 0 && w.R > 0) {
                const int64_t ld = uses_ef(t) ? efw(t) : t.id.dim;
                float* fdst = uses_ef(t) ? w.ef + t.id.dim : w.f;
                if ((rc = launch_add_rows(t.features, t.feat_ld, nullptr, 0, w.R, fo_dim(t), fdst, ld, s, w.fidx)))
                    return rc;
            }
        }
        int maxL = 0;
        for (int k = 0; k < ntowers; ++k)
            if (T[k]->fusion != TTAMM_FUSION_IDENTITY) maxL = T[k]->n_linear > maxL ? T[k]->n_linear : maxL;
        for (int l = 0; l < maxL; ++l) {
            Batcher bb;
            PadSegs pads;
            pads.count = 0;
            for (int k = 0; k < ntowers; ++k) {
                const ttamm_tower& t = *T[k];
                TowerWs& w = *W[k];
                if (t.fusion == TTAMM_FUSION_IDENTITY || l >= t.n_linear) continue;
                const ttamm_linear& L = t.linear[l];
                GemmProblem p = gp_base();
                p.bf16 = t.matmul_bf16;
                if (l == 0) {
                    p.A = t.features;
                    p.a_idx = w.fidx;
                    p.lda = t.feat_ld;
                } else {
                    p.A = w.hid[l - 1];
                    p.lda = t.linear[l - 1].out_features;
                }
                p.B = L.weight;
                p.ldb = L.in_features;
                if (l == 0 && w.w16) {
                    const int kp = round8(L.in_features);
                    if ((rc = launch_to_bf16(L.weight, L.out_features, L.in_features, L.in_features, w.w16, kp, s)))
                        return rc;
                    p.A16 = t.features_bf16;
                    p.lda = t.feat_bf16_ld;
                    p.B16 = w.w16;
                    p.ldb = kp;
                } else if (l == 0 && w.wpad) {
                    pads.seg[pads.count++] = PadSeg{L.weight, L.out_features, L.in_features, L.in_features, w.wpad,
                                                    round4(L.in_features)};
                    p.B = w.wpad;
                    p.ldb = round4(L.in_features);
                }
                p.b_kn = 0;
                p.M = (int)w.R;
                p.N = L.out_features;
                p.K = L.in_features;
                if (l == 0 && w.wpad && t.feat_ld >= round4(L.in_features)) p.K = round4(L.in_features);
                if (l == 0 && w.w16) p.K = round8(L.in_features);
                if (l == 0 && t.features_planes && !t.matmul_bf16 && p.K <= 16 * (t.feat_planes_ld / 48)) {
                    p.A3p = t.features_planes;
                    p.lda3 = t.feat_planes_ld;
                }
                p.bias = L.bias;
                if (l + 1 < t.n_linear) {
                    p.epi = EPI_HIDDEN;
                    p.C = w.hid[l];
                    p.ldc = L.out_features;
                    const uint8_t* injected = w.role == ROLE_USER ? bt.user_keep_mask[l] : bt.item_keep_mask[l];
                    set_dropout(p, t, bt, w.role, l, injected);
                    set_keys(p, w);
                    p.act = t.activation;
                    if (t.activation != TTAMM_ACT_RELU) {
                        p.pre = w.pre[l];
                        if (t.dropout > 0.f && injected == nullptr) p.mask_out = w.mask[l];
                        w.keep[l] = injected ? injected : w.mask[l];
                    }
                } else {
                    p.epi = EPI_STORE;
                    if (uses_ef(t)) {
                        p.C = w.ef + t.id.dim;
                        p.ldc = efw(t);
                    } else {
                        p.C = w.f;
                        p.ldc = D;
                    }
                }
                bb.add(p);
            }
            if ((rc = launch_pad_rows_segs(pads, s))) return rc;
            const bool timed = l == 0 && l0_events && l0_events[0] && l0_events[1];
            if (timed) TTAMM_HIP(hipEventRecord((hipEvent_t)l0_events[0], s));
            if ((rc = bb.run(s))) return rc;
            if (timed) TTAMM_HIP(hipEventRecord((hipEvent_t)l0_events[1], s));
            if (l == 0 && after_l0) TTAMM_HIP(hipEventRecord(after_l0, s));
        }
    }
    return part & FWD_FUSION ? forward_fusion(T, W, D, mimic, s, ntowers) : TTAMM_OK;
}

namespace {
int forward_fusion(const ttamm_tower* T[2], TowerWs* W[2], int D, bool mimic, hipStream_t s, int ntowers) {
    int rc;
    GateArgs ga;
    const bool fused_gate = gate_group(T, W, ntowers, D, mimic, ga);
    if ((rc = require_fused_for_units(T, W, ntowers, fused_gate))) return rc;
    if (fused_gate && ga.count > 0) {
        if ((rc = launch_gate(ga, false, s))) return rc;
        for (int k = 0; k < ntowers; ++k) W[k]->gw16_ready = W[k]->gw16 != nullptr;
    }
    Batcher g1, g2, gc;
    for (int k = 0; k < ntowers; ++k) {
        const ttamm_tower& t = *T[k];
        TowerWs& w = *W[k];
        const float* table = mimic ? t.mimic.weight : nullptr;
        if (t.fusion == TTAMM_FUSION_CONCAT) {
            GemmProblem p = gp_base();
            p.bf16 = t.matmul_bf16;
            p.A = w.ef;
            p.lda = efw(t);
            p.B = t.gate[0].weight;
            p.ldb = efw(t);
            p.M = (int)w.R;
            p.N = D;
            p.K = efw(t);
            p.bias = t.gate[0].bias;
            p.epi = EPI_STORE;
            p.C = w.t;
            p.ldc = w.t_ld;
            gc.add(p);
            continue;
        }
        if (t.fusion == TTAMM_FUSION_GATED) {
            if (fused_gate) continue;
            const int Hg = t.gate[0].out_features;
            GemmProblem p = gp_base();
            p.bf16 = t.matmul_bf16;
            p.A = w.ef;
            p.lda = 2 * D;
            p.B = t.gate[0].weight;
            p.ldb = 2 * D;
            p.M = (int)w.R;
            p.N = Hg;
            p.K = 2 * D;
            p.bias = t.gate[0].bias;
            p.epi = EPI_GATE_HIDDEN;
            p.C = w.z;
            p.ldc = Hg;
            g1.add(p);
            GemmProblem q = gp_base();
            q.bf16 = t.matmul_bf16;
            q.A = w.z;
            q.lda = Hg;
            q.B = t.gate[1].weight;
            q.ldb = Hg;
            q.M = (int)w.R;
            q.N = D;
            q.K = Hg;
            q.bias = t.gate[1].bias;
            if (gate_out_epilogue()) {
                q.epi = EPI_GATE_OUT;
                q.C = w.aug;
                q.ldc = D;
                q.aux0 = w.ef;
                q.ld_aux0 = 2 * D;
                q.out1 = w.g;
                q.out2 = w.t;
                q.out3 = w.a;
                q.table = table;
                q.idx = w.idx;
                q.ld_out = D;
                q.ld_out2 = w.t_ld;
            } else {
                q.epi = EPI_STORE;
                q.C = w.g;
                q.ldc = D;
            }
            g2.add(q);
        } else {
            if ((rc = launch_combine(w.e, D, t.fusion == TTAMM_FUSION_SUM ? w.f : nullptr, D, table, t.mimic.rows, w.idx,
                                     w.R, D, w.t, w.a, w.t_ld, w.aug, s)))
                return rc;
        }
    }
    if ((rc = g1.run(s))) return rc;
    if ((rc = g2.run(s))) return rc;
    if (!gate_out_epilogue() && !fused_gate) {
        for (int k = 0; k < ntowers; ++k) {
            const ttamm_tower& t = *T[k];
            TowerWs& w = *W[k];
            if (t.fusion != TTAMM_FUSION_GATED) continue;
            if ((rc = launch_gate_mix(w.g, w.ef, mimic ? t.mimic.weight : nullptr, w.idx, w.R, D, w.t, w.a, w.t_ld, w.aug, s)))
                return rc;
        }
    }
    if ((rc = gc.run(s))) return rc;
    for (int k = 0; k < ntowers; ++k) {
        const ttamm_tower& t = *T[k];
        TowerWs& w = *W[k];
        if (t.fusion != TTAMM_FUSION_CONCAT) continue;
        if ((rc = launch_combine(w.t, w.t_ld, nullptr, D, mimic ? t.mimic.weight : nullptr, t.mimic.rows, w.idx, w.R,
                                 D, w.t, w.a, w.t_ld, w.aug, s)))
            return rc;
    }
    return TTAMM_OK;
}

bool wgrad_x16() {
    const char* e = dev_env("TTAMM_WGRAD_X16");
    return e && e[0] == '1';
}

int tower_wgrads(const ttamm_tower* T[2], TowerWs* W[2], int D, hipStream_t s, int ntowers, void* const* wg_events);
}

int tower_backward(const ttamm_tower* T[2], TowerWs* W[2], int D, hipStream_t s, int ntowers,
                   void* const* wg_events, int part) {
    int rc;
    if (part & BWD_GATE) {
    GateArgs ga;
    const bool fused_gate = gate_group(T, W, ntowers, D, false, ga);
    if ((rc = require_fused_for_units(T, W, ntowers, fused_gate))) return rc;
    if (fused_gate && ga.count > 0)
        if ((rc = launch_gate(ga, true, s))) return rc;
    Batcher b1, b2;
    for (int k = 0; k < ntowers; ++k) {
        const ttamm_tower& t = *T[k];
        TowerWs& w = *W[k];
        if (t.fusion != TTAMM_FUSION_GATED || fused_gate) continue;
        const int Hg = t.gate[0].out_features;
        if ((rc = launch_gate_dq(w.dT, w.dT_ld, w.ef, w.g, w.R, D, w.dq, s))) return rc;
        GemmProblem p = gp_base();
        p.bf16 = t.matmul_bf16;
        p.A = w.dq;
        p.lda = D;
        p.B = t.gate[1].weight;
        p.ldb = Hg;
        p.b_kn = 1;
        p.M = (int)w.R;
        p.N = Hg;
        p.K = D;
        p.epi = EPI_DGRAD_RELU;
        p.C = w.dz;
        p.ldc = Hg;
        p.aux0 = w.z;
        p.ld_aux0 = Hg;
        b1.add(p);
        GemmProblem q = gp_base();
        q.bf16 = t.matmul_bf16;
        q.A = w.dz;
        q.lda = Hg;
        q.B = t.gate[0].weight;
        q.ldb = 2 * D;
        q.b_kn = 1;
        q.M = (int)w.R;
        q.N = 2 * D;
        q.K = Hg;
        q.epi = EPI_DGRAD_GATE_EF;
        q.C = w.dEF;
        q.ldc = 2 * D;
        q.aux1 = w.dT;
        q.ld_aux1 = w.dT_ld;
        q.aux2 = w.g;
        q.ld_aux2 = D;
        b2.add(q);
    }
    for (int k = 0; k < ntowers; ++k) {
        const ttamm_tower& t = *T[k];
        TowerWs& w = *W[k];
        if (t.fusion != TTAMM_FUSION_CONCAT) continue;
        GemmProblem q = gp_base();
        q.bf16 = t.matmul_bf16;
        q.A = w.dT;
        q.lda = w.dT_ld;
        q.B = t.gate[0].weight;
        q.ldb = efw(t);
        q.b_kn = 1;
        q.M = (int)w.R;
        q.N = efw(t);
        q.K = D;
        q.epi = EPI_STORE;
        q.C = w.dEF;
        q.ldc = efw(t);
        b2.add(q);
    }
    if ((rc = b1.run(s))) return rc;
    if ((rc = b2.run(s))) return rc;
    }
    if (!(part & BWD_MLP)) return TTAMM_OK;
    int maxL = 0;
    for (int k = 0; k < ntowers; ++k)
        if (T[k]->fusion != TTAMM_FUSION_IDENTITY) maxL = T[k]->n_linear > maxL ? T[k]->n_linear : maxL;
    for (int step = 0; step + 1 < maxL; ++step) {
        Batcher bb;
        for (int k = 0; k < ntowers; ++k) {
            const ttamm_tower& t = *T[k];
            TowerWs& w = *W[k];
            if (t.fusion == TTAMM_FUSION_IDENTITY) continue;
            const int l = t.n_linear - 1 - step;
            if (l < 1) continue;
            const ttamm_linear& L = t.linear[l];
            GemmProblem p = gp_base();
            p.bf16 = t.matmul_bf16;
            if (l == t.n_linear - 1) {
                p.A = uses_ef(t) ? w.dEF + t.id.dim : w.dT;
                p.lda = uses_ef(t) ? efw(t) : w.dT_ld;
            } else {
                p.A = w.dhid[l];
                p.lda = L.out_features;
            }
            p.B = L.weight;
            p.ldb = L.in_features;
            p.b_kn = 1;
            p.M = (int)w.R;
            p.N = L.in_features;
            p.K = L.out_features;
            p.epi = EPI_DGRAD_HIDDEN;
            p.C = w.dhid[l - 1];
            p.ldc = L.in_features;
            p.aux0 = w.hid[l - 1];
            p.ld_aux0 = L.in_features;
            const float pdrop = t.dropout;
            p.inv_keep = pdrop > 0.f ? 1.0f / (1.0f - pdrop) : 1.0f;
            p.act = t.activation;
            if (t.activation != TTAMM_ACT_RELU) {
                p.aux0 = w.pre[l - 1];
                p.keep_prob = 1.0f - pdrop;
                p.keep_mask = pdrop > 0.f ? w.keep[l - 1] : nullptr;
            }
            bb.add(p);
        }
        if ((rc = bb.run(s))) return rc;
    }
    return tower_wgrads(T, W, D, s, ntowers, wg_events);
}

namespace {
WgradProblem wgrad_problem(const ttamm_tower& t, const TowerWs& w, const float* dY, int64_t ld_dy, const float* X,
                           int64_t ld_x, int M, int N, float* grad_w, float* grad_b, float* slab) {
    WgradProblem p{};
    p.bf16 = t.matmul_bf16;
    p.dY = dY, p.ld_dy = ld_dy;
    p.X = X, p.ld_x = ld_x;
    p.R = (int)w.R, p.M = M, p.N = N;
    p.grad_w = grad_w, p.grad_b = grad_b, p.slab = slab;
    p.rows_per_split = w.wgrad_rps[wgrad_class(M)];
    return p;
}

int tower_wgrads(const ttamm_tower* T[2], TowerWs* W[2], int D, hipStream_t s, int ntowers, void* const* wg_events) {
    WgradBatch wb;
    std::memset(&wb, 0, sizeof(wb));
    for (int k = 0; k < ntowers; ++k) {
        const ttamm_tower& t = *T[k];
        TowerWs& w = *W[k];
        if (t.fusion == TTAMM_FUSION_IDENTITY) continue;
        float* const* gslab = w.slab + TTAMM_MAX_LINEAR;
        if (t.fusion == TTAMM_FUSION_GATED) {
            const int Hg = t.gate[0].out_features;
            wb.p[wb.count++] = wgrad_problem(t, w, w.dq, D, w.z, Hg, D, Hg, w.ggw[1], w.ggb[1], gslab[1]);
            wb.p[wb.count++] = wgrad_problem(t, w, w.dz, Hg, w.ef, 2 * D, Hg, 2 * D, w.ggw[0], w.ggb[0], gslab[0]);
        }
        if (t.fusion == TTAMM_FUSION_CONCAT)
            wb.p[wb.count++] =
                wgrad_problem(t, w, w.dT, w.dT_ld, w.ef, efw(t), D, efw(t), w.ggw[0], w.ggb[0], gslab[0]);
        for (int l = t.n_linear - 1; l >= 0; --l) {
            const ttamm_linear& L = t.linear[l];
            const bool last = l == t.n_linear - 1;
            const float* dY = !last ? w.dhid[l] : uses_ef(t) ? w.dEF + t.id.dim : w.dT;
            const int64_t ld_dy = !last ? L.out_features : uses_ef(t) ? efw(t) : w.dT_ld;
            WgradProblem p = l == 0 ? wgrad_problem(t, w, dY, ld_dy, t.features, t.feat_ld, L.out_features,
                                                    L.in_features, w.gw[l], w.gb[l], w.slab[l])
                                    : wgrad_problem(t, w, dY, ld_dy, w.hid[l - 1], t.linear[l - 1].out_features,
                                                    L.out_features, L.in_features, w.gw[l], w.gb[l], w.slab[l]);
            if (l == 0) {
                p.x_idx = w.fidx;
                if (uses_w16(t) && wgrad_x16()) {
                    p.X16 = t.features_bf16;
                    p.ld_x16 = t.feat_bf16_ld;
                }
                if (t.features_planes && !t.matmul_bf16) {
                    p.X3p = t.features_planes;
                    p.ld_x3 = t.feat_planes_ld;
                }
            }
            wb.p[wb.count++] = p;
        }
    }
    return launch_wgrad(wb, s, wg_events);
}
}

int stage_ids(const StageSeg* segs, int nsegs, uint32_t* status, const ttamm_tower* const* T, TowerWs* const* W,
              int ntowers, hipStream_t s) {
    int rc;
    StageArgs st;
    std::memset(&st, 0, sizeof(st));
    st.status = status;
    for (int i = 0; i < nsegs; ++i) st.seg[st.count++] = segs[i];
    if ((rc = launch_stage_rows(st, s))) return rc;
    for (int k = 0; k < ntowers; ++k)
        if (W[k]->renorm_mark) {
            TTAMM_HIP(hipMemsetAsync(W[k]->renorm_mark, 0, (size_t)T[k]->id.rows * sizeof(int32_t), s));
            W[k]->renorm_tag = 1;
        }
    return TTAMM_OK;
}

int tower_forward_eval_mode(const ttamm_tower* const* T, TowerWs* const* W, int ntowers, int D, bool mimic,
                            hipStream_t s) {
    ttamm_tower te[2];
    const ttamm_tower* TT[2] = {nullptr, nullptr};
    TowerWs* WW[2] = {nullptr, nullptr};
    for (int k = 0; k < ntowers; ++k) {
        te[k] = *T[k];
        te[k].dropout = 0.f;
        TT[k] = &te[k];
        WW[k] = W[k];
    }
    ttamm_batch bt;
    std::memset(&bt, 0, sizeof(bt));
    return tower_forward(TT, WW, bt, D, mimic, s, ntowers);
}

}
```

Baseline: 13.33 million.

## Skip unneeded gate output rows, fuse dense Adam into wgrad reduce

When in-batch and calibration paths are off, the gate forward stops writing t/a rows past B and aug rows before B, and the score kernels rebuild user/item aug on the fly from t+a. Optionally behind an env flag, the wgrad slab reduction also applies the dense Adam/SGD update in the same kernel, which removes a separate dense update launch and a re-read of the gradients. A configurable unroll depth is added to the slab sum. The point is to cut global memory writes, but score kernels now do extra loads, and the fused path only runs when an env var is set.

New measurement: 13.27 million (median of 2 runs). About the same (-0.5%).

```diff
diff --git a/two-tower-augmented-with-adaptive-mimic-mechanism_amd/csrc/adam.h b/two-tower-augmented-with-adaptive-mimic-mechanism_amd/csrc/adam.h
--- /dev/null
+++ b/two-tower-augmented-with-adaptive-mimic-mechanism_amd/csrc/adam.h
@@ -0,0 +1,70 @@
+#pragma once
+
+#include "kernels.h"
+
+namespace ttamm {
+
+template <bool DECOUPLED, bool G0 = false, bool FAST = false>
+__device__ __forceinline__ void adam_elem_t(float& p, float& m, float& v, float g, const AdamConsts& c) {
+#pragma clang fp contract(off)
+    if (DECOUPLED) {
+        p = p * c.decay;
+    } else if (c.wd != 0.f) {
+        g = g + p * c.wd;
+    }
+    if (G0 && DECOUPLED) {
+        m = fmaf(c.w1, -m, m);
+        v = v * c.b2;
+    } else {
+        m = fmaf(c.w1, g - m, m);
+        v = v * c.b2;
+        v = v + c.w2 * g * g;
+    }
+    if constexpr (FAST) {
+        static_assert(G0, "fast arithmetic is for the g = 0 updates only");
+        const float d = fmaf(__builtin_amdgcn_sqrtf(v), c.fast_ibc, c.fast_eps);
+        p = fmaf(m, __builtin_amdgcn_rcpf(d), p);
+    } else {
+        const float denom = div_by_const(sqrtf(v), c.bc2_sqrt, c.inv_bc2_sqrt) + c.eps;
+        p = p + c.neg_step * (m / denom);
+    }
+}
+
+__device__ __forceinline__ void sgd_elem(float& p, float& m, float& v, float g, const AdamConsts& c) {
+#pragma clang fp contract(off)
+    if (c.wd != 0.f) g = fmaf(p, c.wd, g);
+    if (c.sgd_mom != 0.f) {
+        const float buf = c.sgd_first ? g : fmaf(g, c.sgd_damp1, m * c.sgd_mom);
+        g = c.sgd_nesterov ? fmaf(buf, c.sgd_mom, g) : buf;
+        p = fmaf(g, c.sgd_neg_lr, p);
+        m = v = buf;
+    } else {
+        p = fmaf(g, c.sgd_neg_lr, p);
+        m = v = p;
+    }
+}
+
+__device__ __forceinline__ void adam_elem(float& p, float& m, float& v, float g, const AdamConsts& c) {
+    if (c.sgd)
+        sgd_elem(p, m, v, g, c);
+    else if (c.decoupled)
+        adam_elem_t<true>(p, m, v, g, c);
+    else
+        adam_elem_t<false>(p, m, v, g, c);
+}
+__device__ __forceinline__ void adam_elem_g0(float& p, float& m, float& v, const AdamConsts& c) {
+    if (c.sgd) {
+        sgd_elem(p, m, v, 0.f, c);
+    } else if (c.fast_g0) {
+        if (c.decoupled)
+            adam_elem_t<true, true, true>(p, m, v, 0.f, c);
+        else
+            adam_elem_t<false, true, true>(p, m, v, 0.f, c);
+    } else if (c.decoupled) {
+        adam_elem_t<true, true>(p, m, v, 0.f, c);
+    } else {
+        adam_elem_t<false, true>(p, m, v, 0.f, c);
+    }
+}
+
+}
diff --git a/two-tower-augmented-with-adaptive-mimic-mechanism_amd/csrc/gate.hip b/two-tower-augmented-with-adaptive-mimic-mechanism_amd/csrc/gate.hip
--- a/two-tower-augmented-with-adaptive-mimic-mechanism_amd/csrc/gate.hip
+++ b/two-tower-augmented-with-adaptive-mimic-mechanism_amd/csrc/gate.hip
@@ -143,7 +143,7 @@
 constexpr int slab_scratch() { return 8 * ((D < 96 ? 96 : D) + 4); }
 template <int NO>
 __device__ __forceinline__ void store_slab(float* scr, const f4v (&v)[NO], float* out, int64_t ld, int64_t row0,
-                                           int64_t R, int lane) {
+                                           int64_t R, int lane, int64_t lo = 0) {
     constexpr int W = 16 * NO, LDW = W + 4, C4 = W / 4, PER = 8 * C4 / 64;
     static_assert((8 * C4) % 64 == 0, "slab scratch");
     const int li = lane & 15, q = lane >> 4;
@@ -160,7 +160,7 @@
             const int idx = lane + 64 * k, r = idx / C4, c = idx - r * C4;
             const f4v val = *reinterpret_cast<const f4v*>(scr + r * LDW + 4 * c);
             const int64_t grow = row0 + 8 * half + r;
-            if (grow < R) stg4(out + grow * ld + 4 * c, val);
+            if (grow >= lo && grow < R) stg4(out + grow * ld + 4 * c, val);
         }
         __builtin_amdgcn_s_waitcnt(0xc07f);
         __builtin_amdgcn_wave_barrier();
@@ -346,21 +346,24 @@
                     for (int r = 0; r < 4; ++r) x[ob][r] = neg ? x[ob][r] + a[ob][r] : x[ob][r];
                 store_slab_xu<C::TD>(scr, x, T.t, xu_li, false, s * 16, R, lane);
             } else {
-                store_slab<C::TD>(scr, x, T.t, T.ld_t, s * 16, R, lane);
+                const bool ta = s * 16 < T.ta_rows;
+                if (ta) store_slab<C::TD>(scr, x, T.t, T.ld_t, s * 16, T.ta_rows, lane);
                 if (T.table) {
-                    store_slab<C::TD>(scr, a, T.a, T.ld_t, s * 16, R, lane);
+                    if (ta) store_slab<C::TD>(scr, a, T.a, T.ld_t, s * 16, T.ta_rows, lane);
 #pragma unroll
                     for (int ob = 0; ob < C::TD; ++ob)
 #pragma unroll
                         for (int r = 0; r < 4; ++r) x[ob][r] = x[ob][r] + a[ob][r];
                 }
-                if (T.aug) store_slab<C::TD>(scr, x, T.aug, D, s * 16, R, lane);
+                if (T.aug && s * 16 + 16 > T.aug_from) store_slab<C::TD>(scr, x, T.aug, D, s * 16, R, lane, T.aug_from);
             }
         }
         if ((X || (kDevKnobs && ka->direct)) && ok && !(kDevKnobs && ka->ablate)) {
             const int64_t xu = xu_li;
+            const bool ta = T.xu || row < T.ta_rows;
             float* tdst = T.xu ? T.t + (xu >= 0 ? xu : ~xu) * D : T.t + row * T.ld_t;
-            float* adst = T.xu ? (xu >= 0 ? T.a + xu * D : nullptr) : (T.table ? T.a + row * T.ld_t : nullptr);
+            float* adst = T.xu ? (xu >= 0 ? T.a + xu * D : nullptr) : (T.table && ta ? T.a + row * T.ld_t : nullptr);
+            float* gdst = T.aug && (T.xu || row >= T.aug_from) ? T.aug + row * D : nullptr;
 #pragma unroll
             for (int ob = 0; ob < C::TD; ++ob) {
                 const int col = 16 * ob + 4 * q;
@@ -378,9 +381,9 @@
 #pragma unroll
                     for (int r = 0; r < 4; ++r) aug[r] = tt[r] + a[ob][r];
                 }
-                stg4(tdst + col, T.xu && xu < 0 ? aug : tt);
+                if (ta) stg4(tdst + col, T.xu && xu < 0 ? aug : tt);
                 if (adst) stg4(adst + col, a[ob]);
-                if (T.aug) stg4(T.aug + row * D + col, aug);
+                if (gdst) stg4(gdst + col, aug);
             }
         }
         if constexpr (C::GG) {
diff --git a/two-tower-augmented-with-adaptive-mimic-mechanism_amd/csrc/gemm.hip b/two-tower-augmented-with-adaptive-mimic-mechanism_amd/csrc/gemm.hip
--- a/two-tower-augmented-with-adaptive-mimic-mechanism_amd/csrc/gemm.hip
+++ b/two-tower-augmented-with-adaptive-mimic-mechanism_amd/csrc/gemm.hip
@@ -2,6 +2,7 @@
 #include <cstring>
 #include <type_traits>
 
+#include "adam.h"
 #include "kernels.h"
 
 #ifndef TTAMM_GEMM_ABLATE
@@ -1310,7 +1311,31 @@
     }
 }
 
-__global__ void wgrad_reduce_kernel(WgradBatch batch, int64_t total) {
+template <int NL>
+__device__ __forceinline__ float slab_sum(const float* src, int64_t plane, int splits) {
+    float s = 0.f;
+    int sp = 0;
+    for (; sp + NL <= splits; sp += NL) {
+        float v[NL];
+#pragma unroll
+        for (int i = 0; i < NL; ++i) v[i] = src[(int64_t)(sp + i) * plane];
+#pragma unroll
+        for (int i = 0; i < NL; ++i) s += v[i];
+    }
+    if constexpr (NL > 8) {
+        for (; sp + 8 <= splits; sp += 8) {
+            float v[8];
+#pragma unroll
+            for (int i = 0; i < 8; ++i) v[i] = src[(int64_t)(sp + i) * plane];
+#pragma unroll
+            for (int i = 0; i < 8; ++i) s += v[i];
+        }
+    }
+    for (; sp < splits; ++sp) s += src[(int64_t)sp * plane];
+    return s;
+}
+
+__global__ void wgrad_reduce_kernel(WgradBatch batch, int64_t total, WgradUpdate upd, int update, int depth) {
     const KArg(WgradBatch)* kb = (const KArg(WgradBatch)*)(__builtin_amdgcn_kernarg_segment_ptr());
     const int64_t gid = (int64_t)blockIdx.x * blockDim.x + threadIdx.x;
     if (gid >= total) return;
@@ -1325,19 +1350,26 @@
     const int Mo = P.M;
     const int64_t plane = (int64_t)(P.N + 1) * Mo;
     const int n = (int)(off / Mo), m = (int)(off - (int64_t)n * Mo);
-    float s = 0.f;
+    const bool bias = n >= P.N;
+    float* const gdst = bias ? P.grad_b : P.grad_w;
+    if (!gdst) return;
+    const int64_t o = bias ? (int64_t)m : (int64_t)m * P.N + n;
+    float *pp = nullptr, *pm = nullptr, *pv = nullptr;
+    float p = 0.f, mo = 0.f, v = 0.f;
+    if (update) {
+        pp = (bias ? P.p_b : P.p_w) + o, pm = (bias ? P.m_b : P.m_w) + o, pv = (bias ? P.v_b : P.v_w) + o;
+        p = *pp, mo = *pm, v = *pv;
+    }
     const float* src = P.slab + off;
-    int sp = 0;
-    for (; sp + 8 <= P.splits; sp += 8) {
-        float v[8];
-#pragma unroll
-        for (int i = 0; i < 8; ++i) v[i] = src[(int64_t)(sp + i) * plane];
-#pragma unroll
-        for (int i = 0; i < 8; ++i) s += v[i];
-    }
-    for (; sp < P.splits; ++sp) s += src[(int64_t)sp * plane];
-    if (n < P.N) P.grad_w[(int64_t)m * P.N + n] = s;
-    else if (P.grad_b) P.grad_b[m] = s;
+    const float s = depth >= 32   ? slab_sum<32>(src, plane, P.splits)
+                    : depth >= 16 ? slab_sum<16>(src, plane, P.splits)
+                                  : slab_sum<8>(src, plane, P.splits);
+    gdst[o] = s;
+    if (!update || step_poisoned(upd.status)) return;
+    adam_elem(p, mo, v, s, upd.ad);
+    *pp = p;
+    *pm = mo;
+    *pv = v;
 }
 
 template <class CF, int E, bool BF>
@@ -1668,7 +1700,7 @@
     return on;
 }
 
-int launch_wgrad(WgradBatch& wb, hipStream_t s, void* const* ev) {
+int launch_wgrad(WgradBatch& wb, hipStream_t s, void* const* ev, const WgradUpdate* upd) {
     GemmBatch g[kWgradClasses], gp[kWgradClasses];
     std::memset(g, 0, sizeof(g));
     std::memset(gp, 0, sizeof(gp));
@@ -1715,6 +1747,8 @@
                       "wgrad: rows_per_split must be a multiple of 16 and at most 1024");
         TTAMM_REQUIRE(w.bf16 == wb.p[0].bf16, "wgrad: the batch must share one matmul precision");
         w.splits = w.R > 0 ? (int)ceil_div(w.R, w.rows_per_split) : 1;
+        TTAMM_REQUIRE(!upd || (w.grad_b && w.p_w && w.m_w && w.v_w && w.p_b && w.m_b && w.v_b),
+                      "wgrad: the fused update needs every problem's parameters and moments");
         total += (int64_t)w.M * (w.N + 1);
         if (w.R <= 0) {
             TTAMM_HIP(hipMemsetAsync(w.slab, 0, sizeof(float) * w.M * (w.N + 1), s));
@@ -1782,7 +1816,15 @@
     if (timed) TTAMM_HIP(hipEventRecord((hipEvent_t)ev[1], s));
     if (!narrow_first && ((rc = flush(g[0], 0)) || (rc = flush(gp[0], 0, true)))) return rc;
     if (total > 0) {
-        hipLaunchKernelGGL(wgrad_reduce_kernel, dim3((unsigned)ceil_div(total, 256)), dim3(256), 0, s, wb, total);
+        static const int depth = [] {
+            const char* e = dev_env("TTAMM_WGRAD_REDUCE_DEPTH");
+            return e ? std::atoi(e) : 8;
+        }();
+        WgradUpdate u;
+        std::memset(&u, 0, sizeof(u));
+        if (upd) u = *upd;
+        hipLaunchKernelGGL(wgrad_reduce_kernel, dim3((unsigned)ceil_div(total, 256)), dim3(256), 0, s, wb, total, u,
+                           upd ? 1 : 0, depth);
         TTAMM_LAUNCH_CHECK();
     }
     return TTAMM_OK;
diff --git a/two-tower-augmented-with-adaptive-mimic-mechanism_amd/csrc/kernels.h b/two-tower-augmented-with-adaptive-mimic-mechanism_amd/csrc/kernels.h
--- a/two-tower-augmented-with-adaptive-mimic-mechanism_amd/csrc/kernels.h
+++ b/two-tower-augmented-with-adaptive-mimic-mechanism_amd/csrc/kernels.h
@@ -104,6 +104,8 @@
     int tile_begin;
     int tiles_m, tiles_n;
     int bf16;
+    float *p_w, *m_w, *v_w;
+    float *p_b, *m_b, *v_b;
 };
 constexpr int kMaxWgradProblems = 16;
 static_assert(kMaxWgradProblems >= 2 * (TTAMM_MAX_LINEAR + 2), "both towers: every Linear + the gate's two");
@@ -120,7 +122,8 @@
 int wgrad_class(int m_out);
 void wgrad_rows_per_split(const WgradShape* shapes, int n, int rps[kWgradClasses]);
 size_t wgrad_slab_floats(int R, int M, int N, int rows_per_split);
-int launch_wgrad(WgradBatch& batch, hipStream_t s, void* const* ev = nullptr);
+struct WgradUpdate;
+int launch_wgrad(WgradBatch& batch, hipStream_t s, void* const* ev = nullptr, const WgradUpdate* upd = nullptr);
 
 struct GateTower {
     int64_t R;
@@ -137,6 +140,8 @@
     const float* table;
     const int64_t* idx;
     float* aug;
+    int64_t ta_rows;
+    int64_t aug_from;
     const float* dT;
     int64_t ld_dT;
     const int64_t* xu;
@@ -243,6 +248,7 @@
     int D;
     const float* user_aug;
     const float* item_aug;
+    int item_aug_neg_only;
     const float* t_user;
     const float* t_item;
     const float* a_user;
@@ -482,6 +488,10 @@
     int sgd_first;
     int sgd_nesterov;
 };
+struct WgradUpdate {
+    AdamConsts ad;
+    const uint32_t* status;
+};
 struct SparseConsts {
     float w1;
     float w2;
diff --git a/two-tower-augmented-with-adaptive-mimic-mechanism_amd/csrc/optim.hip b/two-tower-augmented-with-adaptive-mimic-mechanism_amd/csrc/optim.hip
--- a/two-tower-augmented-with-adaptive-mimic-mechanism_amd/csrc/optim.hip
+++ b/two-tower-augmented-with-adaptive-mimic-mechanism_amd/csrc/optim.hip
@@ -6,6 +6,7 @@
 
 #include <type_traits>
 
+#include "adam.h"
 #include "kernels.h"
 
 #pragma clang fp contract(off)
@@ -13,67 +14,6 @@
 namespace ttamm {
 
 namespace {
-
-template <bool DECOUPLED, bool G0 = false, bool FAST = false>
-__device__ __forceinline__ void adam_elem_t(float& p, float& m, float& v, float g, const AdamConsts& c) {
-    if (DECOUPLED) {
-        p = p * c.decay;
-    } else if (c.wd != 0.f) {
-        g = g + p * c.wd;
-    }
-    if (G0 && DECOUPLED) {
-        m = fmaf(c.w1, -m, m);
-        v = v * c.b2;
-    } else {
-        m = fmaf(c.w1, g - m, m);
-        v = v * c.b2;
-        v = v + c.w2 * g * g;
-    }
-    if constexpr (FAST) {
-        static_assert(G0, "fast arithmetic is for the g = 0 updates only");
-        const float d = fmaf(__builtin_amdgcn_sqrtf(v), c.fast_ibc, c.fast_eps);
-        p = fmaf(m, __builtin_amdgcn_rcpf(d), p);
-    } else {
-        const float denom = div_by_const(sqrtf(v), c.bc2_sqrt, c.inv_bc2_sqrt) + c.eps;
-        p = p + c.neg_step * (m / denom);
-    }
-}
-
-__device__ __forceinline__ void sgd_elem(float& p, float& m, float& v, float g, const AdamConsts& c) {
-    if (c.wd != 0.f) g = fmaf(p, c.wd, g);
-    if (c.sgd_mom != 0.f) {
-        const float buf = c.sgd_first ? g : fmaf(g, c.sgd_damp1, m * c.sgd_mom);
-        g = c.sgd_nesterov ? fmaf(buf, c.sgd_mom, g) : buf;
-        p = fmaf(g, c.sgd_neg_lr, p);
-        m = v = buf;
-    } else {
-        p = fmaf(g, c.sgd_neg_lr, p);
-        m = v = p;
-    }
-}
-
-__device__ __forceinline__ void adam_elem(float& p, float& m, float& v, float g, const AdamConsts& c) {
-    if (c.sgd)
-        sgd_elem(p, m, v, g, c);
-    else if (c.decoupled)
-        adam_elem_t<true>(p, m, v, g, c);
-    else
-        adam_elem_t<false>(p, m, v, g, c);
-}
-__device__ __forceinline__ void adam_elem_g0(float& p, float& m, float& v, const AdamConsts& c) {
-    if (c.sgd) {
-        sgd_elem(p, m, v, 0.f, c);
-    } else if (c.fast_g0) {
-        if (c.decoupled)
-            adam_elem_t<true, true, true>(p, m, v, 0.f, c);
-        else
-            adam_elem_t<false, true, true>(p, m, v, 0.f, c);
-    } else if (c.decoupled) {
-        adam_elem_t<true, true>(p, m, v, 0.f, c);
-    } else {
-        adam_elem_t<false, true>(p, m, v, 0.f, c);
-    }
-}
 
 __device__ __forceinline__ void sparse_adam_elem(float& p, float& m, float& v, float g, const SparseConsts& c) {
     const float om = m, ov = v;
diff --git a/two-tower-augmented-with-adaptive-mimic-mechanism_amd/csrc/rows.hip b/two-tower-augmented-with-adaptive-mimic-mechanism_amd/csrc/rows.hip
--- a/two-tower-augmented-with-adaptive-mimic-mechanism_amd/csrc/rows.hip
+++ b/two-tower-augmented-with-adaptive-mimic-mechanism_amd/csrc/rows.hip
@@ -220,9 +220,14 @@
 constexpr int kMaxNeg = 64;
 
 __device__ __forceinline__ float item_aug_at(const ScoreArgs& A, int64_t r, int d, bool neg = false) {
-    if (A.item_aug) return A.item_aug[r * A.ld_item + d];
+    if (A.item_aug && (neg || !A.item_aug_neg_only)) return A.item_aug[r * A.ld_item + d];
     const float t = A.t_item[r * A.ld_item + d];
     return A.a_item && !(neg && A.neg_aug) ? t + A.a_item[r * A.ld_item + d] : t;
+}
+__device__ __forceinline__ float user_aug_at(const ScoreArgs& A, int64_t b, int d) {
+    if (A.user_aug) return A.user_aug[b * A.D + d];
+    const float t = A.t_user[b * A.D + d];
+    return A.a_user ? t + A.a_user[b * A.D + d] : t;
 }
 
 constexpr int kScoreNG = 8;
@@ -248,7 +253,7 @@
             ok[c] = d < D;
             u[c] = p[c] = au[c] = tp[c] = ap[c] = tu[c] = ibp[c] = ibu[c] = 0.f;
             if (ok[c]) {
-                u[c] = A.user_aug[b * D + d];
+                u[c] = user_aug_at(A, b, d);
                 p[c] = item_aug_at(A, pb, d);
                 if (A.mimic) {
                     au[c] = A.a_user[b * D + d];
@@ -382,16 +387,21 @@
     if (b < B) {
         const int64_t pb = A.item_slot ? A.item_slot[b] : b;
         auto item_row = [&](int64_t r, int c, bool neg) {
-            if (A.item_aug) return ld4(A.item_aug + r * ldt + c);
+            if (A.item_aug && (neg || !A.item_aug_neg_only)) return ld4(A.item_aug + r * ldt + c);
             const float4 t = ld4(A.t_item + r * ldt + c);
             return A.a_item && !(neg && A.neg_aug) ? addf4(t, ld4(A.a_item + r * ldt + c)) : t;
         };
+        auto user_row = [&](int c) {
+            if (A.user_aug) return ld4(A.user_aug + b * D + c);
+            const float4 t = ld4(A.t_user + b * D + c);
+            return A.a_user ? addf4(t, ld4(A.a_user + b * D + c)) : t;
+        };
         const float4 z4 = make_float4(0.f, 0.f, 0.f, 0.f);
         float4 u[NV], p[NV], au[NV], tp[NV], ap[NV], tu[NV], ibp[NV], ibu[NV];
 #pragma unroll
         for (int i = 0; i < NV; ++i) {
             const int c = 4 * (s + G * i);
-            u[i] = ld4(A.user_aug + b * D + c);
+            u[i] = user_row(c);
             p[i] = item_row(pb, c, false);
             au[i] = tp[i] = ap[i] = tu[i] = ibp[i] = ibu[i] = z4;
             if (A.mimic) {
diff --git a/two-tower-augmented-with-adaptive-mimic-mechanism_amd/csrc/step.hip b/two-tower-augmented-with-adaptive-mimic-mechanism_amd/csrc/step.hip
--- a/two-tower-augmented-with-adaptive-mimic-mechanism_amd/csrc/step.hip
+++ b/two-tower-augmented-with-adaptive-mimic-mechanism_amd/csrc/step.hip
@@ -573,6 +573,10 @@
                  const float* grad_scale = nullptr) {
     return launch_dense_adam(dense_args(T, W, ad, status, grad_scale), s);
 }
+bool fused_dense_update() {
+    static const bool on = dev_env("TTAMM_FUSED_UPDATE") != nullptr;
+    return on;
+}
 
 int clip_table_partials(Step& c, const StreamPlan& pl, int* off_out) {
     StepWs& ws = c.ws;
@@ -778,7 +782,9 @@
             sa.neg_aug = 1;
         }
     } else {
+        if (U.aug_from > 0) sa.user_aug = nullptr;
         sa.item_aug = I.aug;
+        sa.item_aug_neg_only = I.aug_from > 0 ? 1 : 0;
         sa.t_item = I.t;
         sa.a_item = I.a;
         sa.ld_item = D;
@@ -948,6 +954,11 @@
         I.key_base1 = Bg + A.row_base * N;
         c.neg = I.idx_own + B;
         I.renorm_split = B;
+        static const bool all_rows = dev_env("TTAMM_GATE_ALL_ROWS") != nullptr;
+        if (!c.ws.ib_on && !c.ws.cal_on && !all_rows) {
+            U.aug_from = B;
+            I.ta_rows = I.aug_from = B;
+        }
     }
     U.renorm_tag = I.renorm_tag = (int32_t)(2 * (A.hp.dense_step % (1 << 29)) + 1);
     c.T[0] = &A.user, c.T[1] = &A.item;
@@ -1023,8 +1034,10 @@
     if (single && (rc = loss_finalize(c, pl.aux))) return rc;
     if ((rc = table_updates(c, c.T, c.W, 2, pl, true, A.timing_events))) return rc;
     TTAMM_HIP(hipEventRecord(pl.ev[EV_FROM_AUX], pl.aux));
-    if ((rc = tower_backward(c.T, c.W, c.D, pl.s, 2, A.timing_events + 6, BWD_MLP))) return rc;
-    if (single && (rc = dense_update(c.T, c.W, c.ad, A.status, pl.s))) return rc;
+    const WgradUpdate upd{c.ad, A.status};
+    const bool fused = single && fused_dense_update();
+    if ((rc = tower_backward(c.T, c.W, c.D, pl.s, 2, A.timing_events + 6, BWD_MLP, fused ? &upd : nullptr))) return rc;
+    if (single && !fused && (rc = dense_update(c.T, c.W, c.ad, A.status, pl.s))) return rc;
     TTAMM_HIP(hipStreamWaitEvent(pl.s, pl.ev[EV_FROM_AUX], 0));
     return TTAMM_OK;
 }
diff --git a/two-tower-augmented-with-adaptive-mimic-mechanism_amd/csrc/tower.h b/two-tower-augmented-with-adaptive-mimic-mechanism_amd/csrc/tower.h
--- a/two-tower-augmented-with-adaptive-mimic-mechanism_amd/csrc/tower.h
+++ b/two-tower-augmented-with-adaptive-mimic-mechanism_amd/csrc/tower.h
@@ -34,6 +34,8 @@
     float* a = nullptr;
     int64_t t_ld = 0;
     float* aug = nullptr;
+    int64_t ta_rows = INT64_MAX;
+    int64_t aug_from = 0;
     const float* dT = nullptr;
     float* dT_own = nullptr;
     int64_t dT_ld = 0;
@@ -106,7 +108,7 @@
                   int ntowers, void* const* l0_events = nullptr, int part = FWD_ALL, hipEvent_t after_l0 = nullptr);
 enum { BWD_GATE = 1, BWD_MLP = 2, BWD_ALL = 3 };
 int tower_backward(const ttamm_tower* T[2], TowerWs* W[2], int D, hipStream_t s, int ntowers,
-                   void* const* wg_events = nullptr, int part = BWD_ALL);
+                   void* const* wg_events = nullptr, int part = BWD_ALL, const WgradUpdate* upd = nullptr);
 
 int stage_ids(const StageSeg* segs, int nsegs, uint32_t* status, const ttamm_tower* const* T, TowerWs* const* W,
               int ntowers, hipStream_t s);
diff --git a/two-tower-augmented-with-adaptive-mimic-mechanism_amd/csrc/tower.hip b/two-tower-augmented-with-adaptive-mimic-mechanism_amd/csrc/tower.hip
--- a/two-tower-augmented-with-adaptive-mimic-mechanism_amd/csrc/tower.hip
+++ b/two-tower-augmented-with-adaptive-mimic-mechanism_amd/csrc/tower.hip
@@ -1,3 +1,4 @@
+#include <algorithm>
 #include <cstdint>
 #include <cstring>
 #include <string>
@@ -298,6 +299,8 @@
         g.table = mimic ? t.mimic.weight : nullptr;
         g.idx = w.idx;
         g.aug = w.aug;
+        g.ta_rows = w.xu ? w.R : std::min<int64_t>(w.ta_rows, w.R);
+        g.aug_from = w.xu ? 0 : w.aug_from;
         g.dT = w.dT;
         g.ld_dT = w.dT_ld;
         g.dq = w.dq;
@@ -459,6 +462,9 @@
     GateArgs ga;
     const bool fused_gate = gate_group(T, W, ntowers, D, mimic, ga);
     if ((rc = require_fused_for_units(T, W, ntowers, fused_gate))) return rc;
+    for (int k = 0; k < ntowers; ++k)
+        if (!(fused_gate && ga.planes == 0) || T[k]->fusion != TTAMM_FUSION_GATED || W[k]->xu)
+            W[k]->ta_rows = INT64_MAX, W[k]->aug_from = 0;
     if (fused_gate && ga.count > 0) {
         if ((rc = launch_gate(ga, false, s))) return rc;
         for (int k = 0; k < ntowers; ++k) W[k]->gw16_ready = W[k]->gw16 != nullptr;
@@ -565,11 +571,12 @@
     return e && e[0] == '1';
 }
 
-int tower_wgrads(const ttamm_tower* T[2], TowerWs* W[2], int D, hipStream_t s, int ntowers, void* const* wg_events);
+int tower_wgrads(const ttamm_tower* T[2], TowerWs* W[2], int D, hipStream_t s, int ntowers, void* const* wg_events,
+                 const WgradUpdate* upd);
 }
 
 int tower_backward(const ttamm_tower* T[2], TowerWs* W[2], int D, hipStream_t s, int ntowers,
-                   void* const* wg_events, int part) {
+                   void* const* wg_events, int part, const WgradUpdate* upd) {
     int rc;
     if (part & BWD_GATE) {
     GateArgs ga;
@@ -686,7 +693,7 @@
         }
         if ((rc = bb.run(s))) return rc;
     }
-    return tower_wgrads(T, W, D, s, ntowers, wg_events);
+    return tower_wgrads(T, W, D, s, ntowers, wg_events, upd);
 }
 
 namespace {
@@ -702,9 +709,15 @@
     return p;
 }
 
-int tower_wgrads(const ttamm_tower* T[2], TowerWs* W[2], int D, hipStream_t s, int ntowers, void* const* wg_events) {
+int tower_wgrads(const ttamm_tower* T[2], TowerWs* W[2], int D, hipStream_t s, int ntowers, void* const* wg_events,
+                 const WgradUpdate* upd) {
     WgradBatch wb;
     std::memset(&wb, 0, sizeof(wb));
+    auto add = [&](WgradProblem p, const ttamm_linear& L) {
+        p.p_w = L.weight, p.m_w = L.weight_exp_avg, p.v_w = L.weight_exp_avg_sq;
+        p.p_b = L.bias, p.m_b = L.bias_exp_avg, p.v_b = L.bias_exp_avg_sq;
+        wb.p[wb.count++] = p;
+    };
     for (int k = 0; k < ntowers; ++k) {
         const ttamm_tower& t = *T[k];
         TowerWs& w = *W[k];
@@ -712,12 +725,11 @@
         float* const* gslab = w.slab + TTAMM_MAX_LINEAR;
         if (t.fusion == TTAMM_FUSION_GATED) {
             const int Hg = t.gate[0].out_features;
-            wb.p[wb.count++] = wgrad_problem(t, w, w.dq, D, w.z, Hg, D, Hg, w.ggw[1], w.ggb[1], gslab[1]);
-            wb.p[wb.count++] = wgrad_problem(t, w, w.dz, Hg, w.ef, 2 * D, Hg, 2 * D, w.ggw[0], w.ggb[0], gslab[0]);
+            add(wgrad_problem(t, w, w.dq, D, w.z, Hg, D, Hg, w.ggw[1], w.ggb[1], gslab[1]), t.gate[1]);
+            add(wgrad_problem(t, w, w.dz, Hg, w.ef, 2 * D, Hg, 2 * D, w.ggw[0], w.ggb[0], gslab[0]), t.gate[0]);
         }
         if (t.fusion == TTAMM_FUSION_CONCAT)
-            wb.p[wb.count++] =
-                wgrad_problem(t, w, w.dT, w.dT_ld, w.ef, efw(t), D, efw(t), w.ggw[0], w.ggb[0], gslab[0]);
+            add(wgrad_problem(t, w, w.dT, w.dT_ld, w.ef, efw(t), D, efw(t), w.ggw[0], w.ggb[0], gslab[0]), t.gate[0]);
         for (int l = t.n_linear - 1; l >= 0; --l) {
             const ttamm_linear& L = t.linear[l];
             const bool last = l == t.n_linear - 1;
@@ -738,10 +750,10 @@
                     p.ld_x3 = t.feat_planes_ld;
                 }
             }
-            wb.p[wb.count++] = p;
-        }
-    }
-    return launch_wgrad(wb, s, wg_events);
+            add(p, L);
+        }
+    }
+    return launch_wgrad(wb, s, wg_events, upd);
 }
 }
 
```
